# alexandre01/deepsvg

Hardware: AMD Instinct MI355X
Metric: SVG icons/sec (train step) hierarchical_ordered d=256 (higher is better)
Workload: dtype bf16; 1 GPU; hierarchical_ordered (Hierarchical, use_vae=False) G=8 S=30 d_model=256 ff=512 H=8 L=4x4; full train step = forward + SVGLoss + backward + grad-clip 1.0 + AdamW; dropout 0.1; global_batch=512, batch_per_gpu=512, parallelism=dp1, hip_graph=True, encoder_layout=packed (valid tokens only, exact)

## Files before the change

deepsvg_amd/csrc/gemm.hip:

```cpp
#include "mfma_frag.h"
#include "../../include/dsvg.h"
#include "gemm_common.h"
int dsvg_gemm_group_flush(hipStream_t st);
#include <map>
#include <mutex>
#include <vector>

template <typename T>
__global__ void gemm_naive_kernel(dsvg_gemm_desc p, int k_begin, int k_end, float* part, float* rs) {
    long long idx = (long long)blockIdx.x * blockDim.x + threadIdx.x;
    if (idx >= (long long)p.M * p.N) return;
    int m = (int)(idx / p.N), n = (int)(idx % p.N);
    const T* A = (const T*)p.A;
    const T* B = (const T*)p.B;
    DropCtx adc = drop_make(p.a_drop_p, p.seed, p.a_drop_site);
    float acc = 0.f, asum = 0.f;
    for (int k = k_begin; k < k_end; ++k) {
        float a, b;
        if (p.a_kc) {
            a = Elem<T>::ld(A + (size_t)m * p.lda + k);
            a *= drop_mult(adc, (uint64_t)m * p.a_drop_ld + k);
        } else {
            a = Elem<T>::ld(A + (size_t)k * p.lda + m);
            a *= drop_mult(adc, (uint64_t)k * p.a_drop_ld + m);
// ... 549 lines not shown
    if (int rc = dsvg_gemm_group_flush(st)) return rc;
    if (hipMemsetAsync(out, 0, (size_t)n * sizeof(float), st) != hipSuccess) { dsvg_set_error("defer_zero: hipMemsetAsync failed"); return -1; }
    return 0;
}

int dsvg_reduce_partials_mixed(const float* part, int64_t P, int64_t stride, int64_t n, int64_t n_bf16, float* out,
                               int32_t accumulate, hipStream_t st) {
    if (n <= 0) return 0;
    const bool vec = !(n & 3) && !(stride & 3) && !((uintptr_t)part & 15) && !((uintptr_t)out & 15) && !(n_bf16 & 3);
    {
        DeferTableOfQueues& t = defer_queues();
        std::lock_guard<std::mutex> lk(t.mu);
        auto it = t.by_stream.find(st);
        if (it != t.by_stream.end()) {
            DeferQueue& d = it->second;
            if (!d.q.empty() && defer_overlaps(d, out, n)) {
                int rc = defer_flush_locked(d, st);
                if (rc) return rc;
            }
            static const bool unaligned_ok = !(getenv("DSVG_DEFER_MORE") && atoi(getenv("DSVG_DEFER_MORE")) == 0);
            if (d.scope && (vec || (unaligned_ok && n_bf16 == 0)) && n < (1ll << 30) && P < (1ll << 30)) {
                d.q.push_back(DeferSeg{part, out, (long long)stride, (int)n, (int)n_bf16, (int)P, 0, accumulate, 0});
                return 0;
            }
        }
    }
    if (int rc = dsvg_gemm_group_flush(st)) return rc;
    if (n_bf16 > 0 && !vec) { dsvg_set_error("reduce_partials: bf16 partials need 16-byte aligned, 4-column-multiple data"); return -1; }
    const long long cols = vec ? n / 4 : n;
    const bool wide = cols >= 64 * 128 || P <= 16;
#define DSVG_RP(V, X, B) hipLaunchKernelGGL((reduce_partials_strided_kernel<V, X, B>), dim3(dsvg_cdiv(cols, X)), dim3(256), 0, \
                                            st, part, (long long)P, (long long)stride, (long long)n, out, accumulate,      \
                                            (long long)n_bf16)
    const bool narrow = !vec && n_bf16 == 0 && cols <= 4 && P > 64;
    if (n_bf16 > 0) { if (wide) DSVG_RP(4, 64, true); else DSVG_RP(4, 16, true); }
    else if (vec) { if (wide) DSVG_RP(4, 64, false); else DSVG_RP(4, 16, false); }
    else if (narrow) DSVG_RP(1, 4, false);
    else     { if (wide) DSVG_RP(1, 64, false); else DSVG_RP(1, 16, false); }
#undef DSVG_RP
    DSVG_LAUNCH_CHECK("reduce_partials");
    return 0;
}

constexpr int CS_ROWS_MIN = 16, CS_ROWS_MAX = 1024;
template <typename T>
__global__ __launch_bounds__(256) void colsum_kernel(const T* __restrict__ A, long long lda, long long M, int N,
                                                     float* __restrict__ part, float drop_p, uint32_t site,
                                                     const uint64_t* seed, int cpb, int vec_ok, int rows_per_block) {
    constexpr int VEC = 16 / (int)sizeof(T);
    __shared__ float red[256][VEC + 1];
    const DropCtx dc = drop_make(drop_p, seed, site);
    const int cl = threadIdx.x % cpb, rg = threadIdx.x / cpb, nrg = 256 / cpb;
    const int c0 = (blockIdx.y * cpb + cl) * VEC;
    const long long r0 = (long long)blockIdx.x * rows_per_block;
    const long long r1 = min(M, r0 + rows_per_block);
    float acc[VEC];
#pragma unroll
    for (int e = 0; e < VEC; ++e) acc[e] = 0.f;
    if (c0 < N) {
        if (vec_ok && c0 + VEC <= N) {
            for (long long r = r0 + rg; r < r1; r += nrg) {
                float v[VEC];
                if (VEC == 4) {
                    float t[4];
                    Elem<T>::ld4(A + r * lda + c0, t);
#pragma unroll
                    for (int e = 0; e < 4; ++e) v[e % VEC] = t[e];
                } else {
                    float t0[4], t1[4];
                    Elem<T>::ld4(A + r * lda + c0, t0);
                    Elem<T>::ld4(A + r * lda + c0 + 4, t1);
#pragma unroll
                    for (int e = 0; e < 4; ++e) { v[e] = t0[e]; v[(e + 4) % VEC] = t1[e]; }
                }
                if (VEC == 8 && dc.on && !(N & 7)) {
                    float m8[8];
                    drop_mult8(dc, (uint64_t)r * N + c0, m8);
#pragma unroll
                    for (int e = 0; e < VEC; ++e) acc[e] += v[e] * m8[e % 8];
                } else {
#pragma unroll
                    for (int e = 0; e < VEC; ++e) acc[e] += v[e] * drop_mult(dc, (uint64_t)r * N + c0 + e);
                }
            }
        } else {
            for (long long r = r0 + rg; r < r1; r += nrg)
#pragma unroll
                for (int e = 0; e < VEC; ++e)
                    if (c0 + e < N) acc[e] += Elem<T>::ld(A + r * lda + c0 + e) * drop_mult(dc, (uint64_t)r * N + c0 + e);
        }
    }
#pragma unroll
    for (int e = 0; e < VEC; ++e) red[threadIdx.x][e] = acc[e];
    __syncthreads();
    if (rg == 0 && c0 < N) {
#pragma unroll
        for (int e = 0; e < VEC; ++e) {
            if (c0 + e < N) {
                float s = 0.f;
                for (int g = 0; g < nrg; ++g) s += red[g * cpb + cl][e];
                part[(long long)blockIdx.x * N + c0 + e] = s;
            }
        }
    }
}

extern "C" int64_t dsvg_gemm_workspace_bytes(int32_t M, int32_t N, int32_t split_k) {
    if (split_k <= 1) return 0;
    return (int64_t)split_k * (int64_t)dsvg_splitk_slice(M, N, true) * (int64_t)sizeof(float);
}

extern "C" int dsvg_reduce_partials(const float* partial, int64_t P, int64_t n, float* out,
                                    int32_t accumulate, void* stream) {
    DSVG_CHECK_ARG(partial && out && P >= 0 && n >= 0, "reduce_partials: bad args");
    return dsvg_reduce_partials_strided(partial, P, n, n, out, accumulate, (hipStream_t)stream);
}

extern "C" int64_t dsvg_colsum_workspace_bytes(int64_t M, int32_t N) {
    return (int64_t)dsvg_cdiv(M, CS_ROWS_MIN) * N * (int64_t)sizeof(float);
}

extern "C" int dsvg_colsum(int32_t dtype, const void* A, int64_t lda, int64_t M, int32_t N, float* out,
                           int32_t accumulate, float drop_p, uint32_t drop_site, const uint64_t* seed,
                           float* workspace, int64_t workspace_bytes, void* stream) {
    DSVG_CHECK_ARG(A && out && M > 0 && N > 0, "colsum: bad args");
    DSVG_CHECK_ARG(workspace && workspace_bytes >= dsvg_colsum_workspace_bytes(M, N),
                   "colsum: workspace too small (%lld < %lld)", (long long)workspace_bytes,
                   (long long)dsvg_colsum_workspace_bytes(M, N));
    hipStream_t st = (hipStream_t)stream;
    DSVG_CHECK_ARG(dtype == DSVG_F32 || dtype == DSVG_BF16, "colsum: bad dtype %d", dtype);
    const int vec = dtype == DSVG_F32 ? 4 : 8;
    const int chunks = dsvg_cdiv(N, vec);
    int cpb = 8;
    while (cpb < 64 && cpb < chunks) cpb *= 2;
    const int vec_ok = !(lda % vec) && !((uintptr_t)A & 15);
    const int col_blocks = dsvg_cdiv(chunks, cpb);
    long long rpb = M / max(1, 1024 / col_blocks);
    rpb = rpb < CS_ROWS_MIN ? CS_ROWS_MIN : (rpb > CS_ROWS_MAX ? CS_ROWS_MAX : rpb);
    const int nb = dsvg_cdiv(M, rpb);
    dim3 grid(nb, col_blocks);
    if (dtype == DSVG_F32)
        hipLaunchKernelGGL(colsum_kernel<float>, grid, dim3(256), 0, st, (const float*)A, (long long)lda,
                           (long long)M, N, workspace, drop_p, drop_site, seed, cpb, vec_ok, (int)rpb);
    else
        hipLaunchKernelGGL(colsum_kernel<bf16_t>, grid, dim3(256), 0, st, (const bf16_t*)A, (long long)lda,
                           (long long)M, N, workspace, drop_p, drop_site, seed, cpb, vec_ok, (int)rpb);
    DSVG_LAUNCH_CHECK("colsum");
    return dsvg_reduce_partials(workspace, nb, N, out, accumulate, stream);
}

int dsvg_gemm_bf16_launch(const dsvg_gemm_desc& d, int k_chunk, int nsplit, float* part, float* rs_part,
                          hipStream_t st, int* part_is_bf16);

extern "C" int dsvg_gemm(const dsvg_gemm_desc* dp, void* stream) {
    DSVG_CHECK_ARG(dp, "gemm: null desc");
    dsvg_gemm_desc d = *dp;
    hipStream_t st = (hipStream_t)stream;
    DSVG_CHECK_ARG(d.dtype == DSVG_F32 || d.dtype == DSVG_BF16, "gemm: bad dtype %d", d.dtype);
    DSVG_CHECK_ARG(d.M > 0 && d.N > 0 && d.K > 0, "gemm: bad shape %d %d %d", d.M, d.N, d.K);
    DSVG_CHECK_ARG(d.A && d.B && d.C, "gemm: null operand");
    DSVG_CHECK_ARG((d.drop_p <= 0.f && d.a_drop_p <= 0.f) || d.seed, "gemm: dropout needs a seed pointer");
    if (d.dtype == DSVG_F32) d.c_f32 = 1;
    const int split = d.split_k > 1 ? d.split_k : 1;
    float* part = nullptr;
    int k_chunk = d.K;
    if (split > 1) {
        DSVG_CHECK_ARG(d.c_f32, "gemm: split_k needs fp32 output");
        DSVG_CHECK_ARG(!d.bias && !d.res && !d.gate && d.act == 0 && d.drop_p <= 0.f,
                       "gemm: split_k does not support an epilogue");
        DSVG_CHECK_ARG(d.workspace && d.workspace_bytes >= dsvg_gemm_workspace_bytes(d.M, d.N, split),
                       "gemm: split_k workspace too small");
        DSVG_CHECK_ARG(d.ldc == d.N, "gemm: split_k needs a dense C (ldc == N)");
        part = d.workspace;
        k_chunk = ((d.K + split - 1) / split + 63) / 64 * 64;
    }
    int nsplit = (d.K + k_chunk - 1) / k_chunk;
    if (split > 1 && (split % 8) == 0) nsplit = split;
    DSVG_CHECK_ARG(!d.rowsum || part, "gemm: rowsum needs split_k > 1");
    float* rs_part = d.rowsum ? part + (size_t)d.M * d.N : nullptr;
    const size_t slice = dsvg_splitk_slice(d.M, d.N, d.rowsum != nullptr);

    int part_bf16 = 0;
    bool use_naive = d.impl == 1;
    if (d.dtype == DSVG_F32) {
        if ((d.lda & 3) || (d.ldb & 3) || ((uintptr_t)d.A & 15) || ((uintptr_t)d.B & 15)) use_naive = true;
    } else {
        const int Kp = (d.K + 7) / 8 * 8;
        if ((d.lda & 7) || (d.ldb & 7) || ((uintptr_t)d.A & 15) || ((uintptr_t)d.B & 15)) use_naive = true;
        if ((d.a_kc && d.lda < Kp) || (d.b_kc && d.ldb < Kp)) use_naive = true;
        if (!d.a_kc && d.lda < ((d.M + 7) / 8) * 8) use_naive = true;
        if (!d.b_kc && d.ldb < ((d.N + 7) / 8) * 8) use_naive = true;
    }
    if (use_naive) {
        const long long total = (long long)d.M * d.N;
        for (int z = 0; z < nsplit; ++z) {
            const int kb = z * k_chunk, ke = min(d.K, kb + k_chunk);
            float* pz = part ? part + (size_t)z * slice : nullptr;
            float* rz = rs_part ? rs_part + (size_t)z * slice : nullptr;
            if (d.dtype == DSVG_F32)
                hipLaunchKernelGGL(gemm_naive_kernel<float>, dim3(dsvg_cdiv(total, 256)), dim3(256), 0, st, d, kb, ke, pz, rz);
            else
                hipLaunchKernelGGL(gemm_naive_kernel<bf16_t>, dim3(dsvg_cdiv(total, 256)), dim3(256), 0, st, d, kb, ke, pz, rz);
        }
        DSVG_LAUNCH_CHECK("gemm_naive");
    } else if (d.dtype == DSVG_F32) {
        const int tiles_m = dsvg_cdiv(d.M, BM), tiles_n = dsvg_cdiv(d.N, BN);
        const int nwg = tiles_m * tiles_n;
        dim3 grid(nwg, nsplit);
        if (nsplit > 1 && (nsplit % 8) == 0) grid = dim3(nwg * nsplit, 1);
#define DSVG_F32V(AK, BK)                                                                                              \
    do {                                                                                                               \
        if (rs_part) hipLaunchKernelGGL((gemm_f32_mfma_kernel<AK, BK, true>), grid, dim3(256), 0, st, d, tiles_n, nwg, \
                                        k_chunk, part, rs_part);                                                       \
        else hipLaunchKernelGGL((gemm_f32_mfma_kernel<AK, BK, false>), grid, dim3(256), 0, st, d, tiles_n, nwg,        \
                                k_chunk, part, rs_part);                                                               \
    } while (0)
        if (d.a_kc && d.b_kc) DSVG_F32V(true, true);
        else if (d.a_kc && !d.b_kc) DSVG_F32V(true, false);
        else if (!d.a_kc && d.b_kc) DSVG_F32V(false, true);
        else DSVG_F32V(false, false);
#undef DSVG_F32V
        DSVG_LAUNCH_CHECK("gemm_f32_mfma");
    } else {
        int rc = dsvg_gemm_bf16_launch(d, k_chunk, nsplit, part, rs_part, st, &part_bf16);
        if (rc) return rc;
    }
    if (part && part_bf16) {
        const int64_t mn = (int64_t)d.M * d.N;
        if (rs_part && d.rowsum == (float*)d.C + mn && !(d.M & 3))
            return dsvg_reduce_partials_mixed(part, nsplit, (int64_t)slice, mn + d.M, mn, (float*)d.C, d.accumulate, st);
        int rc = dsvg_reduce_partials_mixed(part, nsplit, (int64_t)slice, mn, mn, (float*)d.C, d.accumulate, st);
        if (rc) return rc;
        if (rs_part) return dsvg_reduce_partials_strided(rs_part, nsplit, (int64_t)slice, d.M, d.rowsum, d.accumulate, st);
        return 0;
    }
    if (part) {
        const int64_t mn = (int64_t)d.M * d.N;
        if (rs_part && d.rowsum == (float*)d.C + mn)
            return dsvg_reduce_partials_strided(part, nsplit, (int64_t)slice, mn + d.M, (float*)d.C, d.accumulate, st);
        int rc = dsvg_reduce_partials_strided(part, nsplit, (int64_t)slice, mn, (float*)d.C, d.accumulate, st);
        if (rc) return rc;
        if (rs_part) return dsvg_reduce_partials_strided(rs_part, nsplit, (int64_t)slice, d.M, d.rowsum, d.accumulate, st);
    }
    return 0;
}
```

deepsvg_amd/csrc/gemm_bf16.h:

```cpp
#pragma once
#include "dsvg_common.h"
#include "../../include/dsvg.h"

enum {
    EPI_GENERIC = 0,
    EPI_BIAS = 1,
    EPI_BIAS_RES_DROP = 2,
    EPI_BIAS_RELU_DROP = 3,
    EPI_GATE = 4,
    EPI_PARTIAL = 5,
};

bool dsvg_gemm_bf16_glds_try(const dsvg_gemm_desc& d, int epi, dim3 grid, int tiles_n, int nwg, int k_chunk,
                             float* part, float* rs_part, int mode, hipStream_t st, int* part_is_bf16);
int dsvg_gemm_group_flush(hipStream_t st);
```

deepsvg_amd/csrc/gemm_bf16_glds.hip:

```cpp
#include "gemm_bf16.h"
#include "mfma_frag.h"
#include <map>
#include <mutex>
#include <vector>

namespace {

constexpr int GBM = 128, GBN = 128, GBK = 64;
constexpr int IMG = 128 * 64;

__device__ __forceinline__ void dma_step8(const char* a0, const char* a1, const char* a2, const char* a3, const char* b0,
                                          const char* b1, const char* b2, const char* b3, uint32_t lds_a, uint32_t lds_b) {
    uint32_t keep;
    asm volatile(
        "s_mov_b32 %0, m0\n\t"
        "s_mov_b32 m0, %9\n\t"
        "s_nop 0\n\t"
        "global_load_lds_dwordx4 %1, off\n\t"
        "s_add_u32 m0, m0, 0x400\n\t"
        "s_nop 0\n\t"
        "global_load_lds_dwordx4 %2, off\n\t"
        "s_add_u32 m0, m0, 0x400\n\t"
        "s_nop 0\n\t"
        "global_load_lds_dwordx4 %3, off\n\t"
        "s_add_u32 m0, m0, 0x400\n\t"
        "s_nop 0\n\t"
        "global_load_lds_dwordx4 %4, off\n\t"
        "s_mov_b32 m0, %10\n\t"
        "s_nop 0\n\t"
        "global_load_lds_dwordx4 %5, off\n\t"
        "s_add_u32 m0, m0, 0x400\n\t"
        "s_nop 0\n\t"
        "global_load_lds_dwordx4 %6, off\n\t"
        "s_add_u32 m0, m0, 0x400\n\t"
        "s_nop 0\n\t"
        "global_load_lds_dwordx4 %7, off\n\t"
        "s_add_u32 m0, m0, 0x400\n\t"
        "s_nop 0\n\t"
        "global_load_lds_dwordx4 %8, off\n\t"
        "s_mov_b32 m0, %0"
        : "=&s"(keep)
        : "v"(a0), "v"(a1), "v"(a2), "v"(a3), "v"(b0), "v"(b1), "v"(b2), "v"(b3), "s"(lds_a), "s"(lds_b)
        : "memory", "scc");
}

template <bool AKC, bool BKC, int EPI, int NST>
__device__ __forceinline__ void glds_body(const dsvg_gemm_desc& p, int tiles_n, int nwg_mn, int k_chunk, float* part,
                                          float* rs_part, int mode, int part_bf16, int bid, int bid_y) {
    __shared__ __attribute__((aligned(1024))) bf16_t smem_static[NST <= 2 ? NST * 2 * IMG : 8];
    extern __shared__ __attribute__((aligned(1024))) bf16_t smem_dynamic[];
    bf16_t* const smem = NST <= 2 ? smem_static : smem_dynamic;

    const int xcd = bid % 8, local = bid / 8;
    int wgid, kz;
    if (mode == 1) {
        wgid = local % nwg_mn;
        kz = (local / nwg_mn) * 8 + xcd;
    } else {
        const int q8 = nwg_mn / 8, r8 = nwg_mn % 8;
        wgid = (xcd < r8 ? xcd * (q8 + 1) : r8 * (q8 + 1) + (xcd - r8) * q8) + local;
        kz = bid_y;
    }
    const int tile_m = wgid / tiles_n, tile_n = wgid % tiles_n;
    const int m0 = tile_m * GBM, n0 = tile_n * GBN;
    const int k_begin = kz * k_chunk;
    const int k_end = min(p.K, k_begin + k_chunk);

    const int tid = threadIdx.x;
    const int lane = tid & 63;
    const int wave = __builtin_amdgcn_readfirstlane(tid >> 6);
    const int wm = wave >> 1, wn = wave & 1;
    const int h = lane >> 5;

    uint32_t offa[4], offb[4];
#pragma unroll
    for (int i = 0; i < 4; ++i) {
        const int piece = wave * 4 + i;
        if (AKC) {
            const int r = piece * 8 + (lane >> 3);
            const int c = (lane & 7) ^ ((r >> 1) & 7);
            offa[i] = (uint32_t)(((size_t)min(m0 + r, p.M - 1) * p.lda + 8 * c) * 2);
        } else {
            const int kr = piece * 4 + (lane >> 4);
            const int c = (lane & 15) ^ ((lane >> 4) << 2);
            offa[i] = (uint32_t)(((size_t)kr * p.lda + min(m0 + 8 * c, ((p.M + 7) & ~7) - 8)) * 2);
        }
        if (BKC) {
            const int r = piece * 8 + (lane >> 3);
            const int c = (lane & 7) ^ ((r >> 1) & 7);
            offb[i] = (uint32_t)(((size_t)min(n0 + r, p.N - 1) * p.ldb + 8 * c) * 2);
        } else {
            const int kr = piece * 4 + (lane >> 4);
            const int c = (lane & 15) ^ ((lane >> 4) << 2);
            offb[i] = (uint32_t)(((size_t)kr * p.ldb + min(n0 + 8 * c, p.N - 8)) * 2);
        }
    }
    auto stage = [&](int k0, int buf) {
        const char* ab = (const char*)p.A + (AKC ? (size_t)k0 * 2 : (size_t)k0 * p.lda * 2);
        const char* bb = (const char*)p.B + (BKC ? (size_t)k0 * 2 : (size_t)k0 * p.ldb * 2);
        bf16_t* da = smem + buf * 2 * IMG + wave * 2048;
        bf16_t* db = da + IMG;
#pragma unroll
        for (int i = 0; i < 4; ++i) {
            __builtin_amdgcn_global_load_lds(DSVG_GLB_PTR(ab + offa[i]), DSVG_LDS_PTR(da + i * 512), 16, 0, 0);
            __builtin_amdgcn_global_load_lds(DSVG_GLB_PTR(bb + offb[i]), DSVG_LDS_PTR(db + i * 512), 16, 0, 0);
        }
    };

    uint32_t fk[4];
#pragma unroll
    for (int kk = 0; kk < 4; ++kk) fk[kk] = (uint32_t)(((lane & 31) * 64 + 8 * ((2 * kk + h) ^ ((lane >> 1) & 7))) * 2);
    const int g = lane >> 4, q = lane & 15;
    auto tr_off = [&](int w, int it) -> uint32_t {
        const int krow = 8 * (g >> 1) + (q >> 2);
        const int chunk = (8 * w + 4 * it + 2 * (g & 1) + ((q & 3) >> 1)) ^ (((q >> 2) & 3) << 2);
        return (uint32_t)((krow * 128 + 8 * chunk + 4 * (q & 1)) * 2);
    };
    const uint32_t ta0 = tr_off(wm, 0), ta1 = tr_off(wm, 1), tb0 = tr_off(wn, 0), tb1 = tr_off(wn, 1);

    auto frag_kc = [&](const char* img, int w, int it, int kk) -> bf16x8 {
        Frag8 f;
        f.u = *reinterpret_cast<const uint4*>(img + (w * 64 + it * 32) * 128 + fk[kk]);
        return f.v;
    };
    auto frag_tr = [&](const char* img, uint32_t off, int kk) -> bf16x8 {
        Frag8 f;
        f.h[0] = __builtin_amdgcn_ds_read_tr16_b64_v4i16((shortx4 __attribute__((address_space(3)))*)(img + off + kk * 4096));
        f.h[1] = __builtin_amdgcn_ds_read_tr16_b64_v4i16(
            (shortx4 __attribute__((address_space(3)))*)(img + off + kk * 4096 + 1024));
        return f.v;
    };

    if (EPI != EPI_PARTIAL && (part_bf16 & 16)) {
        const size_t span = (BKC ? (size_t)p.N * p.ldb : (size_t)p.K * p.ldb) * 2;
        const unsigned n_pc = (unsigned)((span + 4095) >> 12);
        const size_t off = (size_t)(((unsigned)bid >> 3) % n_pc) * 4096 + (size_t)wave * 1024 + (size_t)lane * 16;
        const char* src = (const char*)p.B + (off + 16 <= span ? off : span - 16);
        const uint32_t dst = __builtin_amdgcn_readfirstlane((uint32_t)(uintptr_t)DSVG_LDS_PTR(smem) + (uint32_t)wave * 4096u);
        uint32_t keep;
        asm volatile(
            "s_mov_b32 %0, m0\n\t"
            "s_mov_b32 m0, %2\n\t"
            "s_nop 0\n\t"
            "global_load_lds_dwordx4 %1, off\n\t"
            "s_mov_b32 m0, %0"
            : "=&s"(keep) : "v"(src), "s"(dst) : "memory");
    }

    floatx16 acc00, acc01, acc10, acc11;
#pragma unroll
    for (int r = 0; r < 16; ++r) { acc00[r] = 0.f; acc01[r] = 0.f; acc10[r] = 0.f; acc11[r] = 0.f; }
    const bool do_rs = (EPI == EPI_PARTIAL) && rs_part != nullptr && tile_n == 0;
    float rs0 = 0.f, rs1 = 0.f;
    auto rowsum8 = [](const bf16x8& f, float s) -> float {
        typedef __bf16 bf16x2 __attribute__((ext_vector_type(2)));
        Frag8 t;
        t.v = f;
        const uint32_t w[4] = {t.u.x, t.u.y, t.u.z, t.u.w};
        const bf16x2 one = __builtin_bit_cast(bf16x2, 0x3f803f80u);
#pragma unroll
        for (int e = 0; e < 4; ++e) s = __builtin_amdgcn_fdot2_f32_bf16(__builtin_bit_cast(bf16x2, w[e]), one, s, false);
        return s;
    };

    auto compute = [&](int buf) {
        const char* ia = (const char*)(smem + buf * 2 * IMG);
        const char* ib = ia + IMG * 2;
#pragma unroll
        for (int kk = 0; kk < GBK / 16; ++kk) {
            bf16x8 a0, a1, b0, b1;
            if (AKC) { a0 = frag_kc(ia, wm, 0, kk); a1 = frag_kc(ia, wm, 1, kk); }
            else     { a0 = frag_tr(ia, ta0, kk);   a1 = frag_tr(ia, ta1, kk); }
            if (BKC) { b0 = frag_kc(ib, wn, 0, kk); b1 = frag_kc(ib, wn, 1, kk); }
            else     { b0 = frag_tr(ib, tb0, kk);   b1 = frag_tr(ib, tb1, kk); }
            acc00 = __builtin_amdgcn_mfma_f32_32x32x16_bf16(b0, a0, acc00, 0, 0, 0);
            acc01 = __builtin_amdgcn_mfma_f32_32x32x16_bf16(b0, a1, acc01, 0, 0, 0);
            acc10 = __builtin_amdgcn_mfma_f32_32x32x16_bf16(b1, a0, acc10, 0, 0, 0);
            acc11 = __builtin_amdgcn_mfma_f32_32x32x16_bf16(b1, a1, acc11, 0, 0, 0);
            if (EPI == EPI_PARTIAL && do_rs && (kk >> 1) == wn) { rs0 = rowsum8(a0, rs0); rs1 = rowsum8(a1, rs1); }
        }
    };

    if (NST == 4) {
        const uint32_t lds0 = (uint32_t)(uintptr_t)DSVG_LDS_PTR(smem) + wave * 4096;
        auto issue = [&](int s) {
            const int k0 = k_begin + s * GBK;
            const char* ab = (const char*)p.A + (AKC ? (size_t)k0 * 2 : (size_t)k0 * p.lda * 2);
            const char* bb = (const char*)p.B + (BKC ? (size_t)k0 * 2 : (size_t)k0 * p.ldb * 2);
            const uint32_t la = __builtin_amdgcn_readfirstlane(lds0 + (uint32_t)(s & 3) * (2 * IMG * 2));
            dma_step8(ab + offa[0], ab + offa[1], ab + offa[2], ab + offa[3], bb + offb[0], bb + offb[1], bb + offb[2],
                      bb + offb[3], la, la + IMG * 2);
        };
        const int n_steps = (k_end - k_begin + GBK - 1) / GBK;
        for (int s = 0; s < 3 && s < n_steps; ++s) issue(s);
        for (int s = 0; s < n_steps; ++s) {
            const int ahead = min(n_steps - 1, s + 2) - s;
            if (ahead >= 2) asm volatile("s_waitcnt vmcnt(16)" ::: "memory");
            else if (ahead == 1) asm volatile("s_waitcnt vmcnt(8)" ::: "memory");
            else asm volatile("s_waitcnt vmcnt(0)" ::: "memory");
            __builtin_amdgcn_s_barrier();
            if (s + 3 < n_steps) issue(s + 3);
            compute(s & 3);
        }
    } else if (NST == 1) {
// ... 56 lines not shown
            if (wn == 0 && h == 0) {
                rs0 += rsx[wm * 64 + (lane & 31)];
                rs1 += rsx[wm * 64 + 32 + (lane & 31)];
                if (mrow < p.M) rs_part[(size_t)kz * slice + mrow] = rs0;
                if (mrow + 32 < p.M) rs_part[(size_t)kz * slice + mrow + 32] = rs1;
            }
        }
        return;
    }

    constexpr bool has_res = EPI == EPI_BIAS_RES_DROP;
    constexpr bool has_gate = EPI == EPI_GATE;
    constexpr bool relu = EPI == EPI_BIAS_RELU_DROP;
    constexpr bool may_drop = EPI == EPI_BIAS_RES_DROP || EPI == EPI_BIAS_RELU_DROP;
    const DropCtx dc = drop_make(may_drop ? p.drop_p : 0.f, p.seed, p.drop_site);
    const bool has_bias = !has_gate && p.bias != nullptr;
    const bool bias_al = (reinterpret_cast<uintptr_t>(p.bias) & 15) == 0;
    const bool n_aligned = !(p.N & 7);

    auto tile16 = [&](const floatx16& c, int jn, int im, uint4 (&pk)[2], int (&nvalid)[2]) {
        const int m = mrow + 32 * im;
        uint32_t x[4][4];
#pragma unroll
        for (int gq = 0; gq < 4; ++gq)
#pragma unroll
            for (int e = 0; e < 4; ++e) x[gq][e] = __float_as_uint(c[4 * gq + e]);
#pragma unroll
        for (int e = 0; e < 4; ++e) {
            auto s01 = __builtin_amdgcn_permlane32_swap(x[0][e], x[1][e], false, false);
            auto s23 = __builtin_amdgcn_permlane32_swap(x[2][e], x[3][e], false, false);
            x[0][e] = s01[0]; x[1][e] = s01[1]; x[2][e] = s23[0]; x[3][e] = s23[1];
        }
#pragma unroll
        for (int e = 0; e < 4; ++e) {
            auto s02 = __builtin_amdgcn_permlane32_swap(x[0][e], x[2][e], false, false);
            auto s13 = __builtin_amdgcn_permlane32_swap(x[1][e], x[3][e], false, false);
            x[0][e] = s02[0]; x[2][e] = s02[1]; x[1][e] = s13[0]; x[3][e] = s13[1];
        }
        const int n16 = ncol + 32 * jn + 16 * h;
#pragma unroll
        for (int cb = 0; cb < 2; ++cb) {
            float v[8];
#pragma unroll
            for (int e = 0; e < 4; ++e) { v[e] = __uint_as_float(x[2 * cb][e]); v[4 + e] = __uint_as_float(x[2 * cb + 1][e]); }
            const int nb = n16 + 8 * cb;
            const int nv = (m < p.M && nb < p.N) ? min(8, p.N - nb) : 0;
            nvalid[cb] = nv;
            if (nv == 0) { pk[cb] = make_uint4(0u, 0u, 0u, 0u); continue; }
            if (has_bias) {
                if (nv == 8 && bias_al) {
                    const float4 b0 = *reinterpret_cast<const float4*>(p.bias + nb);
                    const float4 b1 = *reinterpret_cast<const float4*>(p.bias + nb + 4);
                    v[0] += b0.x; v[1] += b0.y; v[2] += b0.z; v[3] += b0.w;
                    v[4] += b1.x; v[5] += b1.y; v[6] += b1.z; v[7] += b1.w;
                } else {
#pragma unroll
                    for (int e = 0; e < 8; ++e) v[e] += e < nv ? p.bias[nb + e] : 0.f;
                }
            }
            if (relu) {
#pragma unroll
                for (int e = 0; e < 8; ++e) v[e] = fmaxf(v[e], 0.f);
            }
            if (has_gate) {
                float gv[8];
                const bf16_t* gp = (const bf16_t*)p.gate + (size_t)m * p.ldgate + nb;
                if (nv == 8) unpack8(*reinterpret_cast<const uint4*>(gp), gv);
                else {
#pragma unroll
                    for (int e = 0; e < 8; ++e) gv[e] = e < nv ? bf2f(gp[e]) : 0.f;
                }
#pragma unroll
                for (int e = 0; e < 8; ++e) v[e] = gv[e] > 0.f ? v[e] * p.gate_scale : 0.f;
            }
            float rv[8];
            if (has_res) {
                const bf16_t* rp = (const bf16_t*)p.res + (size_t)m * p.ldres + nb;
                if (nv == 8) unpack8(*reinterpret_cast<const uint4*>(rp), rv);
                else {
#pragma unroll
                    for (int e = 0; e < 8; ++e) rv[e] = e < nv ? bf2f(rp[e]) : 0.f;
                }
                if (p.res_pre) {
#pragma unroll
                    for (int e = 0; e < 8; ++e) v[e] += rv[e];
                }
            }
            if (may_drop && dc.on) {
                float dm[8];
                if (n_aligned) {
                    drop_mult8(dc, (uint64_t)m * p.N + nb, dm);
                } else {
#pragma unroll
                    for (int e = 0; e < 8; ++e) dm[e] = drop_mult(dc, (uint64_t)m * p.N + nb + e);
                }
#pragma unroll
                for (int e = 0; e < 8; ++e) v[e] *= dm[e];
            }
            if (has_res && !p.res_pre) {
#pragma unroll
                for (int e = 0; e < 8; ++e) v[e] += rv[e];
            }
            pk[cb] = pack8(v);
        }
    };
    auto put8 = [&](bf16_t* cp, const uint4& v, int nv) {
        if (nv == 8) { *reinterpret_cast<uint4*>(cp) = v; return; }
        const uint32_t w[4] = {v.x, v.y, v.z, v.w};
#pragma unroll
        for (int e = 0; e < 8; ++e)
            if (e < nv) cp[e] = (bf16_t)((e & 1) ? (w[e >> 1] >> 16) : (w[e >> 1] & 0xffffu));
    };
    auto row_block = [&](const floatx16& c0, const floatx16& c1, int im) {
        uint4 pk0[2], pk1[2];
        int nv0[2], nv1[2];
        tile16(c0, 0, im, pk0, nv0);
        tile16(c1, 1, im, pk1, nv1);
        bf16_t* cp = (bf16_t*)p.C + (size_t)(mrow + 32 * im) * p.ldc + ncol + 16 * h;
        put8(cp, pk0[0], nv0[0]);
        put8(cp + 8, pk0[1], nv0[1]);
        put8(cp + 32, pk1[0], nv1[0]);
        put8(cp + 40, pk1[1], nv1[1]);
    };
    row_block(acc00, acc10, 0);
    row_block(acc01, acc11, 1);
}

template <bool AKC, bool BKC, int EPI, int NST, int OCC>
__global__ __launch_bounds__(256, NST == 1 ? OCC : 2) void gemm_bf16_glds_kernel(dsvg_gemm_desc p, int tiles_n, int nwg_mn,
                                                                              int k_chunk, float* part, float* rs_part,
                                                                              int mode, int part_bf16) {
    glds_body<AKC, BKC, EPI, NST>(p, tiles_n, nwg_mn, k_chunk, part, rs_part, mode, part_bf16, (int)blockIdx.x, (int)blockIdx.y);
}

constexpr int GROUP_MAX = 16;
struct WgItem {
    const void* A; const void* B; float* part; float* rs_part;
    int M, N, K, tiles_n, nwg_mn, k_chunk, mode, part_bf16, first_block, grid_x;
    long long lda, ldb;
};
struct WgTable { WgItem it[GROUP_MAX]; int n; };
static_assert(sizeof(WgTable) <= 3600, "the problem table must fit the kernel-argument segment");

__global__ __launch_bounds__(256, 2) void gemm_bf16_wgrad_group_kernel(const WgTable t) {
    int g = 0;
    while (g + 1 < t.n && (int)blockIdx.x >= t.it[g + 1].first_block) ++g;
    const WgItem& w = t.it[g];
    dsvg_gemm_desc p;
    p.A = w.A; p.B = w.B; p.M = w.M; p.N = w.N; p.K = w.K; p.lda = w.lda; p.ldb = w.ldb;
    const int local = (int)blockIdx.x - w.first_block;
    glds_body<false, false, EPI_PARTIAL, 4>(p, w.tiles_n, w.nwg_mn, w.k_chunk, w.part, w.rs_part, w.mode, w.part_bf16,
                                            local % w.grid_x, local / w.grid_x);
}

struct GroupQueue {
    int scope = 0;
    std::vector<WgItem> q;
};
struct GroupQueues {
    std::mutex mu;
    std::map<hipStream_t, GroupQueue> by_stream;
};
GroupQueues& group_queues() { static GroupQueues g; return g; }

int group_launch_locked(GroupQueue& gq, hipStream_t st) {
    size_t at = 0;
    while (at < gq.q.size()) {
        WgTable t;
        int blocks = 0, k = 0;
        for (; k < GROUP_MAX && at < gq.q.size(); ++k, ++at) {
            t.it[k] = gq.q[at];
            t.it[k].first_block = blocks;
            blocks += gq.q[at].first_block;
        }
        t.n = k;
        const size_t lds = (size_t)4 * 2 * IMG * sizeof(bf16_t);
        static bool once = false;
        if (!once) {
            (void)hipFuncSetAttribute((const void*)gemm_bf16_wgrad_group_kernel, hipFuncAttributeMaxDynamicSharedMemorySize,
                                      (int)lds);
            once = true;
        }
        hipLaunchKernelGGL(gemm_bf16_wgrad_group_kernel, dim3(blocks), dim3(256), lds, st, t);
    }
    gq.q.clear();
    return 0;
}

template <bool AKC, bool BKC, int EPI>
void launch(const dsvg_gemm_desc& d, dim3 grid, int tiles_n, int nwg, int k_chunk, float* part, float* rs_part, int mode,
            int nst, hipStream_t st, int pbf = 0) {
    static const int occ = getenv("DSVG_GEMM_OCC") ? atoi(getenv("DSVG_GEMM_OCC")) : 4;
    static const int w_warm = getenv("DSVG_GEMM_WARM") ? atoi(getenv("DSVG_GEMM_WARM")) : 0;
    if (EPI != EPI_PARTIAL && w_warm) pbf |= 16;
    if (nst == 4) {
        const size_t lds = (size_t)4 * 2 * IMG * sizeof(bf16_t);
        static bool once = false;
        if (!once) {
            (void)hipFuncSetAttribute((const void*)gemm_bf16_glds_kernel<AKC, BKC, EPI, 4, 4>,
                                      hipFuncAttributeMaxDynamicSharedMemorySize, (int)lds);
            once = true;
        }
        hipLaunchKernelGGL((gemm_bf16_glds_kernel<AKC, BKC, EPI, 4, 4>), grid, dim3(256), lds, st, d, tiles_n, nwg, k_chunk,
                           part, rs_part, mode, pbf);
    } else if (nst == 2)
        hipLaunchKernelGGL((gemm_bf16_glds_kernel<AKC, BKC, EPI, 2, 4>), grid, dim3(256), 0, st, d, tiles_n, nwg, k_chunk,
                           part, rs_part, mode, pbf);
    else if (occ == 5)
        hipLaunchKernelGGL((gemm_bf16_glds_kernel<AKC, BKC, EPI, 1, 5>), grid, dim3(256), 0, st, d, tiles_n, nwg, k_chunk,
                           part, rs_part, mode, pbf);
    else
        hipLaunchKernelGGL((gemm_bf16_glds_kernel<AKC, BKC, EPI, 1, 4>), grid, dim3(256), 0, st, d, tiles_n, nwg, k_chunk,
                           part, rs_part, mode, pbf);
}

}

bool dsvg_gemm_bf16_glds_try(const dsvg_gemm_desc& d, int epi, dim3 grid, int tiles_n, int nwg, int k_chunk, float* part,
                             float* rs_part, int mode, hipStream_t st, int* part_is_bf16) {
    static const bool pbf_on = !(getenv("DSVG_SPLITK_BF16") && atoi(getenv("DSVG_SPLITK_BF16")) == 0);
    static const bool disabled = getenv("DSVG_GEMM_NOGLDS") != nullptr;
    static const int nst_env = getenv("DSVG_GEMM_STAGES") ? atoi(getenv("DSVG_GEMM_STAGES")) : 1;
    if (disabled || d.impl == 2 || mode == 2 || d.a_drop_p > 0.f) return false;
    static const int deep_wgs = getenv("DSVG_GEMM_DEEP_WGS") ? atoi(getenv("DSVG_GEMM_DEEP_WGS")) : 256;
    const long long n_wgs = (long long)grid.x * grid.y * grid.z;
    const int nst = d.impl == 6 ? 4 : (d.impl == 3 ? 2 : (d.impl == 4 ? 1 : (n_wgs <= deep_wgs ? 4 : nst_env)));
    if ((d.K % GBK) || (part && (k_chunk % GBK))) return false;
    if ((d.lda & 7) || (d.ldb & 7) || ((uintptr_t)d.A & 15) || ((uintptr_t)d.B & 15)) return false;
    if (!d.a_kc && d.M < 8) return false;
    if (!d.b_kc && ((d.N & 7) || d.N < 8)) return false;
    if (d.M < 1 || d.N < 1) return false;
    const size_t span_a = d.a_kc ? (size_t)d.M * d.lda : (size_t)GBK * d.lda + d.M;
    const size_t span_b = d.b_kc ? (size_t)d.N * d.ldb : (size_t)GBK * d.ldb + d.N;
    if (span_a * 2 >= (1ull << 32) || span_b * 2 >= (1ull << 32)) return false;
    if (part) {
        if (((uintptr_t)part & 15) || (d.N & 3)) return false;
        if (!d.a_kc && !d.b_kc) {
            const int pbf = (pbf_on && part_is_bf16 && !(d.N & 7)) ? 1 : 0;
            if (nst == 4 && grid.z == 1) {
                GroupQueues& G = group_queues();
                std::lock_guard<std::mutex> lk(G.mu);
                auto it = G.by_stream.find(st);
                if (it != G.by_stream.end() && it->second.scope) {
                    WgItem w;
                    w.A = d.A; w.B = d.B; w.part = part; w.rs_part = rs_part;
                    w.M = d.M; w.N = d.N; w.K = d.K; w.tiles_n = tiles_n; w.nwg_mn = nwg; w.k_chunk = k_chunk; w.mode = mode;
                    w.part_bf16 = pbf; w.first_block = (int)(grid.x * grid.y); w.grid_x = (int)grid.x;
                    w.lda = d.lda; w.ldb = d.ldb;
                    it->second.q.push_back(w);
                    if (part_is_bf16) *part_is_bf16 = pbf;
                    return true;
                }
            }
            launch<false, false, EPI_PARTIAL>(d, grid, tiles_n, nwg, k_chunk, part, rs_part, mode, nst, st, pbf);
            if (part_is_bf16) *part_is_bf16 = pbf;
            return true;
        }
        return false;
    }
    if (d.bias && ((uintptr_t)d.bias & 3)) return false;
    if (d.a_kc && d.b_kc) {
        if (epi == EPI_BIAS) launch<true, true, EPI_BIAS>(d, grid, tiles_n, nwg, k_chunk, part, rs_part, mode, nst, st);
        else if (epi == EPI_BIAS_RES_DROP) launch<true, true, EPI_BIAS_RES_DROP>(d, grid, tiles_n, nwg, k_chunk, part, rs_part, mode, nst, st);
        else if (epi == EPI_BIAS_RELU_DROP) launch<true, true, EPI_BIAS_RELU_DROP>(d, grid, tiles_n, nwg, k_chunk, part, rs_part, mode, nst, st);
        else return false;
        return true;
    }
    if (d.a_kc && !d.b_kc) {
        if (epi == EPI_BIAS) launch<true, false, EPI_BIAS>(d, grid, tiles_n, nwg, k_chunk, part, rs_part, mode, nst, st);
        else if (epi == EPI_GATE) launch<true, false, EPI_GATE>(d, grid, tiles_n, nwg, k_chunk, part, rs_part, mode, nst, st);
        else return false;
        return true;
    }
    return false;
}

int dsvg_gemm_group_flush(hipStream_t st) {
    GroupQueues& G = group_queues();
    std::lock_guard<std::mutex> lk(G.mu);
    auto it = G.by_stream.find(st);
    if (it == G.by_stream.end() || it->second.q.empty()) return 0;
    const int rc = group_launch_locked(it->second, st);
    hipError_t e = hipGetLastError();
    if (e != hipSuccess) { dsvg_set_error("gemm group: launch failed: %s", hipGetErrorString(e)); return -2; }
    return rc;
}

extern "C" int dsvg_gemm_group_scope(int32_t on, void* stream) {
    hipStream_t st = (hipStream_t)stream;
    {
        GroupQueues& G = group_queues();
        std::lock_guard<std::mutex> lk(G.mu);
        if (on) { G.by_stream[st].scope = 1; return 0; }
        auto it = G.by_stream.find(st);
        if (it == G.by_stream.end()) return 0;
        it->second.scope = 0;
    }
    const int rc = dsvg_gemm_group_flush(st);
    {
        GroupQueues& G = group_queues();
        std::lock_guard<std::mutex> lk(G.mu);
        auto it = G.by_stream.find(st);
        if (it != G.by_stream.end() && it->second.q.empty() && !it->second.scope) G.by_stream.erase(it);
    }
    return rc;
}
```

deepsvg_amd/csrc/layernorm.hip:

```cpp
#include "dsvg_common.h"
#include "../../include/dsvg.h"

constexpr int LN_MAXV_MAX = 4;
constexpr int LN_MAX_BLOCKS = 1024;

template <typename T, int LN_MAXV>
__global__ __launch_bounds__(256) void ln_fwd_kernel(const T* __restrict__ x, const float* __restrict__ gamma,
                                                     const float* __restrict__ beta, T* __restrict__ y,
                                                     float* __restrict__ mean, float* __restrict__ rstd,
                                                     long long rows, int d, float eps) {
    const int lane = threadIdx.x & 63;
    const int wave = threadIdx.x >> 6;
    const int nv = d / 256 + ((d % 256) ? 1 : 0);
    float4 g4[LN_MAXV], b4[LN_MAXV];
#pragma unroll
    for (int i = 0; i < LN_MAXV; ++i) {
        const int c = min(i * 256 + lane * 4, d - 4);
        g4[i] = *reinterpret_cast<const float4*>(gamma + c);
        b4[i] = *reinterpret_cast<const float4*>(beta + c);
    }
    for (long long row = (long long)blockIdx.x * 4 + wave; row < rows; row += (long long)gridDim.x * 4) {
        const T* xr = x + row * d;
        float v[LN_MAXV][4];
        float s = 0.f;
#pragma unroll
        for (int i = 0; i < LN_MAXV; ++i) {
            const int c = i * 256 + lane * 4;
            if (i < nv && c < d) {
                Elem<T>::ld4(xr + c, v[i]);
                s += v[i][0] + v[i][1] + v[i][2] + v[i][3];
            } else {
                v[i][0] = v[i][1] = v[i][2] = v[i][3] = 0.f;
            }
        }
        const float mu = wave_sum(s) / (float)d;
        float s2 = 0.f;
#pragma unroll
        for (int i = 0; i < LN_MAXV; ++i) {
            const int c = i * 256 + lane * 4;
            if (i < nv && c < d) {
#pragma unroll
                for (int e = 0; e < 4; ++e) { const float t = v[i][e] - mu; s2 += t * t; }
            }
        }
        const float var = wave_sum(s2) / (float)d;
        const float rs = rsqrtf(var + eps);
        if (lane == 0) { mean[row] = mu; rstd[row] = rs; }
        T* yr = y + row * d;
#pragma unroll
        for (int i = 0; i < LN_MAXV; ++i) {
            const int c = i * 256 + lane * 4;
            if (i < nv && c < d) {
                const float4 g = g4[i];
                const float4 b = b4[i];
                float o[4];
                o[0] = (v[i][0] - mu) * rs * g.x + b.x;
                o[1] = (v[i][1] - mu) * rs * g.y + b.y;
                o[2] = (v[i][2] - mu) * rs * g.z + b.z;
                o[3] = (v[i][3] - mu) * rs * g.w + b.w;
                Elem<T>::st4(yr + c, o);
            }
        }
    }
}

template <typename T, int LN_MAXV>
__global__ __launch_bounds__(256) void ln_bwd_kernel(const T* dy, const T* __restrict__ x,
                                                     const float* __restrict__ mean, const float* __restrict__ rstd,
                                                     const float* __restrict__ gamma, const T* res,
                                                     T* dx, float* __restrict__ part,
                                                     long long rows, int d, T* dxm, float drop_p,
                                                     const uint64_t* __restrict__ seed, uint32_t site) {
    const DropCtx dmc = drop_make(dxm ? drop_p : 0.f, seed, site);
    extern __shared__ float red_raw[];
    const int nvec = d / 4 + 1;
    auto red = [&](int w, int k, int vec, int e) -> float& { return red_raw[((w * 2 + k) * nvec + vec) * 4 + e]; };
    const int lane = threadIdx.x & 63;
    const int wave = threadIdx.x >> 6;
    const int nv = d / 256 + ((d % 256) ? 1 : 0);
    float ag[LN_MAXV][4], ab[LN_MAXV][4];
#pragma unroll
    for (int i = 0; i < LN_MAXV; ++i)
#pragma unroll
        for (int e = 0; e < 4; ++e) { ag[i][e] = 0.f; ab[i][e] = 0.f; }

    float4 g4[LN_MAXV];
#pragma unroll
    for (int i = 0; i < LN_MAXV; ++i) g4[i] = *reinterpret_cast<const float4*>(gamma + min(i * 256 + lane * 4, d - 4));
    for (long long row = (long long)blockIdx.x * 4 + wave; row < rows; row += (long long)gridDim.x * 4) {
        const float mu = mean[row], rs = rstd[row];
        float xh[LN_MAXV][4], gd[LN_MAXV][4], rv[LN_MAXV][4];
        float c1 = 0.f, c2 = 0.f;
#pragma unroll
        for (int i = 0; i < LN_MAXV; ++i) {
            const int c = i * 256 + lane * 4;
            if (i < nv && c < d) {
                float xv[4], dv[4];
                Elem<T>::ld4(x + row * d + c, xv);
                Elem<T>::ld4(dy + row * d + c, dv);
                if (res) Elem<T>::ld4(res + row * d + c, rv[i]);
                const float4 g = g4[i];
                const float gg[4] = {g.x, g.y, g.z, g.w};
#pragma unroll
                for (int e = 0; e < 4; ++e) {
                    xh[i][e] = (xv[e] - mu) * rs;
                    gd[i][e] = gg[e] * dv[e];
                    c1 += gd[i][e];
                    c2 += gd[i][e] * xh[i][e];
                    ag[i][e] += dv[e] * xh[i][e];
                    ab[i][e] += dv[e];
                }
            } else {
#pragma unroll
                for (int e = 0; e < 4; ++e) { xh[i][e] = 0.f; gd[i][e] = 0.f; }
            }
        }
        c1 = wave_sum(c1) / (float)d;
        c2 = wave_sum(c2) / (float)d;
#pragma unroll
        for (int i = 0; i < LN_MAXV; ++i) {
            const int c = i * 256 + lane * 4;
            if (i < nv && c < d) {
                float o[4];
#pragma unroll
                for (int e = 0; e < 4; ++e) o[e] = rs * (gd[i][e] - c1 - xh[i][e] * c2);
                if (res) {
#pragma unroll
                    for (int e = 0; e < 4; ++e) o[e] += rv[i][e];
                }
                Elem<T>::st4(dx + row * d + c, o);
                if (dxm) {
                    const uint64_t id4 = (uint64_t)row * (uint64_t)d + (uint64_t)c;
                    float mm[4] = {1.f, 1.f, 1.f, 1.f};
                    if (dmc.on) {
                        const uint32_t hg = drop_group(dmc, id4 >> 3);
                        const uint32_t wb = ((uint32_t)id4 & 4u) ? 2u : 0u;
                        const uint32_t w0 = drop_word(hg, wb), w1 = drop_word(hg, wb + 1u);
                        mm[0] = (w0 & 0xffffu) < dmc.thresh ? 0.f : dmc.scale;
                        mm[1] = (w0 >> 16) < dmc.thresh ? 0.f : dmc.scale;
                        mm[2] = (w1 & 0xffffu) < dmc.thresh ? 0.f : dmc.scale;
                        mm[3] = (w1 >> 16) < dmc.thresh ? 0.f : dmc.scale;
                    }
                    float om[4];
#pragma unroll
                    for (int e = 0; e < 4; ++e) {
                        T t;
                        Elem<T>::st(&t, o[e]);
                        om[e] = Elem<T>::ld(&t) * mm[e];
                    }
                    Elem<T>::st4(dxm + row * d + c, om);
                }
            }
        }
    }
#pragma unroll
    for (int i = 0; i < LN_MAXV; ++i) {
        if (i < nv) {
#pragma unroll
            for (int e = 0; e < 4; ++e) {
                if (i * 256 + lane * 4 < d) {
                    red(wave, 0, i * 64 + lane, e) = ag[i][e];
                    red(wave, 1, i * 64 + lane, e) = ab[i][e];
                }
            }
        }
    }
    __syncthreads();
    float* pg = part + (size_t)blockIdx.x * 2 * d;
    for (int c = threadIdx.x; c < d; c += 256) {
        const int vec = c >> 2, e = c & 3;
        float sg = 0.f, sb = 0.f;
#pragma unroll
        for (int w = 0; w < 4; ++w) { sg += red(w, 0, vec, e); sb += red(w, 1, vec, e); }
        pg[c] = sg;
        pg[d + c] = sb;
    }
}

static int ln_grid(long long rows) {
    static const int cap = getenv("DSVG_LN_BLOCKS") ? atoi(getenv("DSVG_LN_BLOCKS")) : LN_MAX_BLOCKS;
    long long nb = (rows + 3) / 4;
    return (int)(nb < cap ? nb : cap);
}
static int ln_grid_fwd(long long rows) {
    long long nb = (rows + 3) / 4;
    return (int)(nb < 65536 ? nb : 65536);
}

extern "C" int dsvg_layernorm_fwd(int32_t dtype, const void* x, const float* gamma, const float* beta, void* y,
                                  float* mean, float* rstd, int64_t rows, int32_t d, float eps, void* stream) {
    DSVG_CHECK_ARG(x && gamma && beta && y && mean && rstd, "layernorm_fwd: null pointer");
    DSVG_CHECK_ARG(rows > 0 && d > 0 && (d % 4) == 0 && d <= 1024, "layernorm_fwd: bad shape rows=%lld d=%d",
                   (long long)rows, d);
    hipStream_t st = (hipStream_t)stream;
#define DSVG_LNF(TT, NV) hipLaunchKernelGGL((ln_fwd_kernel<TT, NV>), dim3(ln_grid_fwd(rows)), dim3(256), 0, st, \
                                            (const TT*)x, gamma, beta, (TT*)y, mean, rstd, (long long)rows, d, eps)
    if (dtype == DSVG_F32) { if (d <= 256) DSVG_LNF(float, 1); else if (d <= 512) DSVG_LNF(float, 2); else DSVG_LNF(float, 4); }
    else if (dtype == DSVG_BF16) { if (d <= 256) DSVG_LNF(bf16_t, 1); else if (d <= 512) DSVG_LNF(bf16_t, 2); else DSVG_LNF(bf16_t, 4); }
    else { dsvg_set_error("layernorm_fwd: bad dtype %d", dtype); return -1; }
#undef DSVG_LNF
    DSVG_LAUNCH_CHECK("layernorm_fwd");
    return 0;
}

extern "C" int64_t dsvg_layernorm_bwd_workspace_bytes(int64_t rows, int32_t d) {
    return (int64_t)ln_grid(rows) * 2 * d * (int64_t)sizeof(float);
}

static int ln_bwd_launch(int32_t dtype, const void* dy, const void* x, const float* mean, const float* rstd,
                         const float* gamma, const void* res, void* dx, float* dgamma, float* dbeta,
                         int32_t accumulate, int64_t rows, int32_t d, float* workspace,
                         int64_t workspace_bytes, void* dx_masked, float drop_p, uint32_t drop_site, const void* seed,
                         void* stream);

extern "C" int dsvg_layernorm_bwd(int32_t dtype, const void* dy, const void* x, const float* mean, const float* rstd,
                                  const float* gamma, const void* res, void* dx, float* dgamma, float* dbeta,
                                  int32_t accumulate, int64_t rows, int32_t d, float* workspace,
                                  int64_t workspace_bytes, void* stream) {
    return ln_bwd_launch(dtype, dy, x, mean, rstd, gamma, res, dx, dgamma, dbeta, accumulate, rows, d, workspace,
                         workspace_bytes, nullptr, 0.f, 0u, nullptr, stream);
}

extern "C" int dsvg_layernorm_bwd_masked(int32_t dtype, const void* dy, const void* x, const float* mean, const float* rstd,
                                         const float* gamma, const void* res, void* dx, float* dgamma, float* dbeta,
                                         int32_t accumulate, int64_t rows, int32_t d, float* workspace,
                                         int64_t workspace_bytes, void* dx_masked, float drop_p, uint32_t drop_site,
                                         const void* seed, void* stream) {
    DSVG_CHECK_ARG(dx_masked && dx_masked != dx, "layernorm_bwd_masked: needs a second output buffer");
    DSVG_CHECK_ARG(!(drop_p > 0.f) || seed, "layernorm_bwd_masked: dropout needs a seed");
    return ln_bwd_launch(dtype, dy, x, mean, rstd, gamma, res, dx, dgamma, dbeta, accumulate, rows, d, workspace,
                         workspace_bytes, dx_masked, drop_p, drop_site, seed, stream);
}

static int ln_bwd_launch(int32_t dtype, const void* dy, const void* x, const float* mean, const float* rstd,
                         const float* gamma, const void* res, void* dx, float* dgamma, float* dbeta,
                         int32_t accumulate, int64_t rows, int32_t d, float* workspace,
                         int64_t workspace_bytes, void* dx_masked, float drop_p, uint32_t drop_site, const void* seed,
                         void* stream) {
    DSVG_CHECK_ARG(dy && x && mean && rstd && gamma && dx && dgamma && dbeta, "layernorm_bwd: null pointer");
    DSVG_CHECK_ARG(rows > 0 && d > 0 && (d % 4) == 0 && d <= 1024, "layernorm_bwd: bad shape");
    DSVG_CHECK_ARG(workspace && workspace_bytes >= dsvg_layernorm_bwd_workspace_bytes(rows, d),
                   "layernorm_bwd: workspace too small");
    hipStream_t st = (hipStream_t)stream;
    const int nb = ln_grid(rows);
    const size_t lds = (size_t)4 * 2 * (d / 4 + 1) * 4 * sizeof(float);
#define DSVG_LNB(TT, NV) hipLaunchKernelGGL((ln_bwd_kernel<TT, NV>), dim3(nb), dim3(256), lds, st, (const TT*)dy, \
                                            (const TT*)x, mean, rstd, gamma, (const TT*)res, (TT*)dx, workspace,  \
                                            (long long)rows, d, (TT*)dx_masked, drop_p, (const uint64_t*)seed, drop_site)
    if (dtype == DSVG_F32) { if (d <= 256) DSVG_LNB(float, 1); else if (d <= 512) DSVG_LNB(float, 2); else DSVG_LNB(float, 4); }
    else if (dtype == DSVG_BF16) { if (d <= 256) DSVG_LNB(bf16_t, 1); else if (d <= 512) DSVG_LNB(bf16_t, 2); else DSVG_LNB(bf16_t, 4); }
    else { dsvg_set_error("layernorm_bwd: bad dtype %d", dtype); return -1; }
#undef DSVG_LNB
    DSVG_LAUNCH_CHECK("layernorm_bwd");
    if (dbeta == dgamma + d)
        return dsvg_reduce_partials_strided(workspace, nb, 2 * (int64_t)d, 2 * (int64_t)d, dgamma, accumulate, st);
    int rc = 0;
    rc = dsvg_reduce_partials_strided(workspace, nb, 2 * (int64_t)d, d, dgamma, accumulate, st);
    if (rc) return rc;
    rc = dsvg_reduce_partials_strided(workspace + d, nb, 2 * (int64_t)d, d, dbeta, accumulate, st);
    return rc;
}
```

deepsvg_amd/functional.py:

```python
import math
import contextlib
import functools
import os

import torch

from . import ops

FFN_MIN_ROWS = int(os.environ.get("DSVG_FFN_MIN_ROWS", "16384"))
ATTN_MIN_ROWS = int(os.environ.get("DSVG_ATTN_MIN_ROWS", "16384"))
FFN_GATE_DW2 = os.environ.get("DSVG_FFN_GATE_DW2", "1") != "0"

LN_BWD_MASKED = os.environ.get("DSVG_LN_BWD_MASKED", "1") != "0"
DEFER_MORE = os.environ.get("DSVG_DEFER_MORE", "1") != "0"
HEAD_KPAD = os.environ.get("DSVG_HEAD_KPAD", "1") != "0"
GS_STACK = os.environ.get("DSVG_GS_STACK", "1") != "0"
_ATTN_VALU = os.environ.get("DSVG_ATTN_VALU") is not None
_ATTN_MFMA_MIN_S = int(os.environ.get("DSVG_ATTN_MFMA_MIN_S", "2"))
GS_REMAINDER = int(os.environ.get("DSVG_GS_REMAINDER", "512"))
SEQ_ROUND = 2048
HEAD_FUSED = os.environ.get("DSVG_HEAD_FUSED", "0") != "0"

_NULL_CTX = contextlib.nullcontext()

class Runtime:

    def __init__(self, dtype=torch.float32, seed=None, store=None, training=False, defer=False):
        self.dtype = dtype
        self.defer = bool(defer)
        self.seed = seed
        self.store = store
        self.training = training
        self.masked = {}
        self.last_layer_gs = False
        self.stack_group = None
        self.path_stage = False
        self.cond_grad = {}

    def cond_grad_block(self, z, rows):
        if z is None or z.dim() != 2 or z.stride(1) != 1 or z.dtype != torch.bfloat16:
            return None
        w, ld = z.shape[1], z.stride(0)
        if ld <= w or ld % w or w % 8 or w > 512:
            return None
        i = (z.storage_offset() % ld) // w
        if (z.storage_offset() % ld) % w:
            return None
        base = z.data_ptr() - i * w * z.element_size()
        key = (base, rows, ld)
        buf = self.cond_grad.get(key)
        if buf is None:
            if len(self.cond_grad) > 8:
                self.cond_grad.clear()
            buf = self.cond_grad[key] = torch.empty((rows, ld), dtype=z.dtype, device=z.device)
        return buf[:, i * w:(i + 1) * w]

    def deferring(self):
        return ops.DEFER if self.defer else _NULL_CTX

    def stack_group_begin(self):
        if self.stack_group is None:
            ops.GROUP.__enter__()
            self.stack_group = []
        return self.stack_group

    def stack_group_end(self):
        if self.stack_group is not None:
            ops.GROUP.__exit__(None, None, None)
            self.stack_group = None

    def deferring_tables(self):
        return ops.DEFER if self.defer and DEFER_MORE else _NULL_CTX

    def grouping(self):
        return ops.GROUP

    def p(self, rate):
        return float(rate) if (self.training and rate > 0.0) else 0.0

    def w(self, param):
        if self.dtype == torch.float32:
            return param.detach()
        if self.store is not None:
            v = self.store.lp(param)
            if v is not None:
                return v
        return param.detach().to(self.dtype)

    def grad_out(self, param):
        if self.store is not None:
            v = self.store.grad_view(param)
            if v is not None:
                return v
        return torch.empty(param.shape, dtype=torch.float32, device=param.device)


def _wgrad_tag():
    return ops.tag_default("wgrad") if ops.PROFILE_ON else _NULL_CTX


def _wgrad(rt, param, dy, x, *, a_drop_p=0.0, a_drop_site=0):
    out = rt.grad_out(param)
    n_out, k_in = param.shape
    T = dy.shape[0]
    with rt.deferring(), _wgrad_tag():
        ops.gemm(dy, x, a_kc=False, b_kc=False, out=out.view(n_out, k_in), a_drop_p=a_drop_p, a_drop_site=a_drop_site,
                 seed=rt.seed, split_k=ops.split_k_for(n_out, k_in, T))
    return out


def _wbgrad(rt, weight, bias, dy, x, blocks=None, *, out=None, split=None, defer=True):
    if split is None:
        split = ops.split_k_for(*weight.shape, dy.shape[0], target_blocks=blocks)
    dw, db = out if out is not None else (rt.grad_out(weight), rt.grad_out(bias))
    with (rt.deferring() if defer else _NULL_CTX), _wgrad_tag():
        if split > 1:
            ops.gemm(dy, x, a_kc=False, b_kc=False, out=dw, split_k=split, rowsum=db)
        else:
            ops.gemm(dy, x, a_kc=False, b_kc=False, out=dw)
            ops.colsum(dy, out=db)
    return dw, db


def _group_blocks(w):
    return 8 * -(-w.shape[0] // 128) * -(-w.shape[1] // 128)


def _bgrad(rt, param, dy, *, drop_p=0.0, drop_site=0):
    out = rt.grad_out(param)
    with rt.deferring():
        ops.colsum(dy, out=out, drop_p=drop_p, drop_site=drop_site, seed=rt.seed)
    return out


def _hand_masked(rt, dx, dxm, p, site):
    if len(rt.masked) > 8:
        rt.masked.clear()
    rt.masked[dx.data_ptr()] = (dxm, p, site, dx._version)


def _take_masked(rt, dx, p, site, rows=None):
    hit = rt.masked.pop(dx.data_ptr(), None)
    if hit is None:
        return None
    dxm, hp, hsite, ver = hit
    n = dx.shape[0] if rows is None else rows
    if (hp != p or hsite != site or dxm.dtype != dx.dtype or dxm.shape[0] < n or dxm.shape[1:] != dx.shape[1:]
            or dx._version != ver):
        return None
    return dxm[:n]


def _aligned2d(t, mult):
    if t.dim() == 2 and t.stride(1) == 1 and t.stride(0) % mult == 0 and t.data_ptr() % 16 == 0:
        return t
    rows, cols = t.shape
    ld = (cols + mult - 1) // mult * mult
    buf = torch.zeros((rows, ld), dtype=t.dtype, device=t.device)
    buf[:, :cols].copy_(t)
    return buf[:, :cols]


class LinearFn(torch.autograd.Function):

    @staticmethod
    def forward(ctx, rt, x, weight, bias, act, res, drop_rate, site, out_dtype):
        p = rt.p(drop_rate)
        dt = out_dtype or x.dtype
        n_out = weight.shape[0]
        mult = 4 if dt == torch.float32 else 8
        out = None
        if n_out % mult:
            ld = (n_out + mult - 1) // mult * mult
            out = torch.empty((x.shape[0], ld), dtype=dt, device=x.device)[:, :n_out]
        y = ops.gemm(x, rt.w(weight), bias=bias.detach() if bias is not None else None, act=act,
                     res=res, drop_p=p, drop_site=site, seed=rt.seed, out_dtype=out_dtype, out=out)
        ctx.rt, ctx.act, ctx.p, ctx.site = rt, act, p, site
        ctx.has_res = res is not None
        ctx.save_for_backward(x, weight, bias, y if act == ops.RELU else None)
        return y

    @staticmethod
    def backward(ctx, dy):
        rt = ctx.rt
        x, weight, bias, y = ctx.saved_tensors
        mult = 4 if rt.dtype == torch.float32 else 8
        dy = _aligned2d(dy.to(rt.dtype) if dy.dtype != rt.dtype else dy, mult)
        dres = dy if ctx.has_res else None
        if ctx.act == ops.RELU:
            assert not ctx.has_res, "relu with a fused residual cannot be differentiated from the saved output"
            scale = ops.keep_scale(ctx.p)
            dy_eff, a_drop_p_eff, a_site = ops.gate_mul(dy.contiguous(), y, scale), 0.0, 0
        else:
            dy_eff, a_drop_p_eff, a_site = dy, ctx.p, ctx.site
        dx = None
        if ctx.needs_input_grad[1]:
            dx = ops.gemm(dy_eff, rt.w(weight), b_kc=False, a_drop_p=a_drop_p_eff, a_drop_site=a_site, seed=rt.seed)
        if a_drop_p_eff == 0.0 and bias is not None:
            dw, db = _wbgrad(rt, weight, bias, dy_eff, x)
        else:
            dw = _wgrad(rt, weight, dy_eff, x, a_drop_p=a_drop_p_eff, a_drop_site=a_site)
            db = _bgrad(rt, bias, dy_eff, drop_p=a_drop_p_eff, drop_site=a_site) if bias is not None else None
        return None, dx, dw, db, None, dres, None, None, None


class ResBlockFn(torch.autograd.Function):

    @staticmethod
    def forward(ctx, rt, z, weight, bias):
        r = ops.gemm(z, rt.w(weight), bias=bias.detach(), act=ops.RELU)
        ctx.rt = rt
        ctx.save_for_backward(z, r, weight, bias)
        return ops.add(z, r)

    @staticmethod
    def backward(ctx, dout):
        rt = ctx.rt
        z, r, weight, bias = ctx.saved_tensors
        dout = dout.contiguous()
        dpre = ops.gate_mul(dout, r, 1.0)
        dw, db = _wbgrad(rt, weight, bias, dpre, z)
        dz = ops.gemm(dpre, rt.w(weight), b_kc=False, res=dout)
        return None, dz, dw, db


LATENT_FUSED = os.environ.get("DSVG_LATENT_FUSED", "1") != "0"


class LatentChainFn(torch.autograd.Function):

    @staticmethod
    def forward(ctx, rt, z, *wb):
        ws = [rt.w(w) for w in wb[0::2]]
        bs = [b.detach() for b in wb[1::2]]
        ctx.rt, ctx.n = rt, len(ws) - 1
        z = z.contiguous()
        if any(ctx.needs_input_grad):
            out, zs, rs = ops.latent_chain_fwd(z, ws, bs, train=True)
            ctx.save_for_backward(z, *zs, *rs, *wb)
        else:
            out = ops.latent_chain_fwd(z, ws, bs)
        return out

    @staticmethod
    def backward(ctx, dout):
        rt, n = ctx.rt, ctx.n
        saved = ctx.saved_tensors
        zin = [saved[0]] + list(saved[1:1 + n])
        rs = list(saved[1 + n:1 + 2 * n])
        wb = saved[1 + 2 * n:]
        dout = dout.contiguous()
        dz0, dpre = ops.latent_chain_bwd(dout, [rt.w(w) for w in wb[0::2]], rs)
        grads = []
        with rt.grouping():
            for i in range(n + 1):
                w, b = wb[2 * i], wb[2 * i + 1]
                grads += list(_wbgrad(rt, w, b, dpre[i] if i < n else dout, zin[i], _group_blocks(w)))
        return (None, dz0, *grads)


class LivePrefix(tuple):
    armed = False


def _live_rows(live, full_rows):
    if live is None or live[1] >= full_rows:
        return None
    return live


def _armed(live):
    if live is None or not getattr(live, "armed", True):
        return None
    return live
# ... 415 lines not shown
            xn1, mean1, rstd1 = ops.layernorm_fwd(x, n1w.detach(), n1b.detach())
            qkv = ops.gemm(xn1, rt.w(win), bias=bin_.detach())
            if causal:
                ao = ops.attention_fwd(qkv, key_mask, n_seq, S, n_heads, scale, p, site0, rt.seed, causal=True)
            else:
                ao = ops.attention_fwd(qkv, key_mask, n_seq, S, n_heads, scale, p, site0, rt.seed, seq_off=seq_off,
                                       tiles=tiles, **_path_kw(rt, S))
            x1 = ops.gemm(ao, rt.w(wo), bias=bo.detach(), res=x, drop_p=p, drop_site=site0 + 1, seed=rt.seed)
        ctx.tiles, ctx.causal = tiles, causal
        if z is not None and not z_fused:
            g = z.contiguous() if wg is None else ops.gemm(z, rt.w(wg), bias=bg.detach())
            ops.bcast_add_fwd_(x1, g, n_seq, S, p, site0 + 2, rt.seed)
        if l is not None:
            g2 = ops.gemm(l, rt.w(wg2), bias=bg2.detach())
            ops.bcast_add_fwd_(x1, g2, n_seq, S, p, site0 + 5, rt.seed)
        ffn = rt.store.ffn(w1) if (rt.store is not None and x.dtype == torch.bfloat16 and x.shape[0] >= FFN_MIN_ROWS) else None
        ctx.ffn_fused = ffn is not None
        if split:
            pass
        elif ffn is not None:
            mean2 = rstd2 = None
            with ops.tag("ffn"):
                if want_bwd:
                    x2, h, xn2, _rstd = ops.ffn_fwd(x1, ffn[0], ffn[2], b2.detach(), 1e-5, p, site0 + 3, site0 + 4, rt.seed,
                                                    train=True)
                else:
                    xn2 = h = None
                    x2 = ops.ffn_fwd(x1, ffn[0], ffn[2], b2.detach(), 1e-5, p, site0 + 3, site0 + 4, rt.seed)
        else:
            with ops.tag("ffn"):
                xn2, mean2, rstd2 = ops.layernorm_fwd(x1, n2w.detach(), n2b.detach())
                h = ops.gemm(xn2, rt.w(w1), bias=b1.detach(), act=ops.RELU, drop_p=p, drop_site=site0 + 3, seed=rt.seed)
                x2 = ops.gemm(h, rt.w(w2), bias=b2.detach(), res=x1, drop_p=p, drop_site=site0 + 4, seed=rt.seed)
        ctx.rt, ctx.n_seq, ctx.S, ctx.n_heads, ctx.p, ctx.site0, ctx.scale = rt, n_seq, S, n_heads, p, site0, scale
        assert seq_off is None or (z is None and l is None), "packed layout: no per-sequence conditioning adds"
        ctx.live = _live_rows(live, x.shape[0])
        assert ctx.live is None or (seq_off is None and key_mask is None and l is None)
        ctx.save_for_backward(x, key_mask, z, l, mean1, rstd1, xn1, qkv, ao, x1, mean2, rstd2, xn2, h,
                              n1w, n1b, win, bin_, wo, bo, n2w, n2b, w1, b1, w2, b2, wg, bg, wg2, bg2, seq_off)
        return x2

    @staticmethod
    def backward(ctx, dx2):
        rt, n_seq, S, H, p, s0 = ctx.rt, ctx.n_seq, ctx.S, ctx.n_heads, ctx.p, ctx.site0
        (x, key_mask, z, l, mean1, rstd1, xn1, qkv, ao, x1, mean2, rstd2, xn2, h,
         n1w, n1b, win, bin_, wo, bo, n2w, n2b, w1, b1, w2, b2, wg, bg, wg2, bg2, seq_off) = ctx.saved_tensors
        dx2 = dx2.contiguous()
        full_rows, n_seq_full = x.shape[0], n_seq
        live = _armed(ctx.live)
        dx2_masked = _take_masked(rt, dx2, p, s0 + 4, rows=(live[1] if live is not None else None)) if p > 0 else None
        if live is not None:
            n_seq, R = live
            (dx2, x, mean1, rstd1, xn1, qkv, ao, x1, mean2, rstd2, xn2, h) = (
                (t[:R] if t is not None else None) for t in (dx2, x, mean1, rstd1, xn1, qkv, ao, x1, mean2, rstd2, xn2, h))
        inv_keep = ops.keep_scale(p)
        dx1m = None
        if ctx.gs:
            gs = rt.store.gs(win)
            with rt.deferring(), ops.tag("gs"):
                (dx, dx1, dym, dpre, dx1m, dqkv, dn2w, dn2b, dn1w, dn1b, *dg_) = ops.gs_layer_bwd(
                    dx2, gs[1], x, mean1, rstd1, qkv, x1, mean2, rstd2, h, n1w.detach(), n2w.detach(), key_mask, n_seq, S,
                    ctx.scale, p, s0, rt.seed, want_dx1=False, dgamma2=rt.grad_out(n2w),
                    dbeta2=rt.grad_out(n2b), dgamma1=rt.grad_out(n1w), dbeta1=rt.grad_out(n1b), want_dg=z is not None)
            dz = dg = None
            if z is not None:
                dg = dg_[0]
                if wg is None:
                    dz = dg
                elif ctx.needs_input_grad[3]:
                    dz = ops.gemm(dg, rt.w(wg), b_kc=False)
            (dw2, db2), (dw1, db1), (dwo, dbo), (dwin, dbin), (dwg, dbg) = _gs_queue_wgrads(
                rt, ctx.first_in_stack, (w2, b2, dym, h), (w1, b1, dpre, xn2), (wo, bo, dx1m, ao), (win, bin_, dqkv, xn1),
                cond=(wg if z is not None else None, bg, dg, z))
            return (None, dx, None, dz, None, None, None, None, None, None,
                    dn1w, dn1b, dwin, dbin, dwo, dbo, dn2w, dn2b, dw1, db1, dw2, db2, dwg, dbg, None, None, None, None, None,
                    None, None, None)
        if ctx.ffn_fused:
            pb, _b1f, w2p = rt.store.ffn(w1)[1:]
            T = x1.shape[0]
            with ops.tag("ffn"):
                g2p = torch.empty((256, 512), dtype=torch.float32, device=x1.device)
                g1p = torch.empty((512, 256), dtype=torch.float32, device=x1.device)
                db1p = torch.empty(512, dtype=torch.float32, device=x1.device)
                db2 = rt.grad_out(b2)
                s2, s1 = ops.split_k_for(256, 512, T), ops.split_k_for(512, 256, T)
                hp, xh = h, xn2
                dym = dx2_masked if dx2_masked is not None else ops.drop_apply(dx2, p, s0 + 4, rt.seed)
                if (FFN_GATE_DW2 and s2 > 1 and dym.is_cuda and dym.dtype == torch.bfloat16
                        and dym.is_contiguous() and hp.is_contiguous() and w2p.is_contiguous()):
                    with rt.deferring():
                        dpre = ops.ffn_gate_dw2(dym, hp, w2p, inv_keep, g2p, db2, s2)
                else:
                    _wbgrad(rt, None, None, dym, hp, out=(g2p, db2), split=s2)
                    dpre = ops.gemm(dym, w2p, b_kc=False, gate=hp, gate_scale=inv_keep)
                _wbgrad(rt, None, None, dpre, xh, out=(g1p, db1p), split=s1)
                dx1 = ops.ffn_bwd_dx(dpre, x1, dx2, pb)
                dw1, db1, dw2 = rt.grad_out(w1), rt.grad_out(b1), rt.grad_out(w2)
                dn2w, dn2b = rt.grad_out(n2w), rt.grad_out(n2b)
                fin = (g1p, db1p, g2p, w1.detach(), n2w.detach(), n2b.detach(), dw1.detach(), db1.detach(), dw2.detach(),
                       dn2w.detach(), dn2b.detach())
                if rt.defer:
                    ops.ffn_wgrad_finish_deferred(*fin)
                else:
                    ops.ffn_wgrad_finish(*fin)
            del hp, dpre, xh, dym
        else:
            with ops.tag("ffn"):
                dx2m = dx2_masked if dx2_masked is not None else ops.drop_apply(dx2, p, s0 + 4, rt.seed)
                dw2, db2 = _wbgrad(rt, w2, b2, dx2m, h)
                dh = ops.gemm(dx2m, rt.w(w2), b_kc=False, gate=h, gate_scale=inv_keep)
                dw1, db1 = _wbgrad(rt, w1, b1, dh, xn2)
                dxn2 = ops.gemm(dh, rt.w(w1), b_kc=False)
                with rt.deferring():
                    dx1, dn2w, dn2b = ops.layernorm_bwd(dxn2, x1, mean2, rstd2, n2w.detach(), res=dx2,
                                                        dgamma=rt.grad_out(n2w), dbeta=rt.grad_out(n2b))
            del dx2m
        dz = dl = dwg = dbg = dwg2 = dbg2 = None
        if l is not None:
            dg2 = ops.bcast_add_bwd(dx1, n_seq, S, p, s0 + 5, rt.seed)
            dwg2, dbg2 = _wbgrad(rt, wg2, bg2, dg2, l)
            if ctx.needs_input_grad[4]:
                dl = ops.gemm(dg2, rt.w(wg2), b_kc=False)
        if z is not None:
            vec = dx1.dtype == torch.bfloat16 and dx1.is_contiguous() and dx1.shape[1] % 8 == 0 and dx1.shape[1] <= 512
            dg_out = rt.cond_grad_block(z, n_seq_full) if (wg is None and vec and dx1.data_ptr() % 16 == 0) else None
            if p > 0 and vec and n_seq * S <= dx1.shape[0] <= n_seq_full * S:
                dg, dx1m = ops.bcast_add_bwd(dx1, n_seq, S, p, s0 + 2, rt.seed, n_seq_out=n_seq_full, mask_site=s0 + 1, out=dg_out)
            else:
                dg = ops.bcast_add_bwd(dx1, n_seq, S, p, s0 + 2, rt.seed, n_seq_out=n_seq_full, out=dg_out)
            if wg is None:
                dz = dg
            else:
                dwg, dbg = _wbgrad(rt, wg, bg, dg, z)
                if ctx.needs_input_grad[3]:
                    dz = ops.gemm(dg, rt.w(wg), b_kc=False)
        if dx1m is None:
            dx1m = ops.drop_apply(dx1, p, s0 + 1, rt.seed)
        dwo, dbo = _wbgrad(rt, wo, bo, dx1m, ao)
        wob = None
        if (not _ATTN_VALU and S >= _ATTN_MFMA_MIN_S and _attn_fused_eligible(rt, x, x.shape[0], key_mask, H, ctx.causal)
                and ((seq_off is None and 16 < S <= 32 and x.shape[0] >= n_seq * S) or (seq_off is not None and ctx.tiles is not None))):
            wob = rt.store.attn_bwd(win)
        if wob is not None:
            dqkv = ops.attention_bwd_outproj(qkv, key_mask, dx1m, wob, n_seq, S, ctx.scale, p, s0, rt.seed, seq_off=seq_off,
                                             tiles=ctx.tiles)
        else:
            dao = ops.gemm(dx1m, rt.w(wo), b_kc=False)
            if ctx.causal:
                dqkv = ops.attention_bwd(qkv, key_mask, dao, n_seq, S, H, ctx.scale, p, s0, rt.seed, causal=True)
            else:
                dqkv = ops.attention_bwd(qkv, key_mask, dao, n_seq, S, H, ctx.scale, p, s0, rt.seed, seq_off=seq_off,
                                         tiles=ctx.tiles, **_path_kw(rt, S))
        del dx1m
        dwin, dbin = _wbgrad(rt, win, bin_, dqkv, xn1)
        dx_out = None
        if live is not None:
            dx_full = torch.empty((full_rows, x.shape[1]), dtype=x.dtype, device=x.device)
            dx_out = dx_full[:x.shape[0]]
        mk = (p, ctx.mask_below, rt.seed) if (ctx.mask_below is not None and p > 0) else None
        with rt.deferring():
            dxn1 = ops.gemm(dqkv, rt.w(win), b_kc=False)
            out = ops.layernorm_bwd(dxn1, x, mean1, rstd1, n1w.detach(), res=dx1, dx=dx_out,
                                    dgamma=rt.grad_out(n1w), dbeta=rt.grad_out(n1b), masked=mk)
            dx, dn1w, dn1b = out[:3]
        if live is not None:
            dx = dx_full
        if mk is not None:
            _hand_masked(rt, dx, out[3], p, ctx.mask_below)
        return (None, dx, None, dz, dl, None, None, None, None, None,
                dn1w, dn1b, dwin, dbin, dwo, dbo, dn2w, dn2b, dw1, db1, dw2, db2, dwg, dbg, dwg2, dbg2, None, None, None,
                None, None, None)


def gs_stack_eligible(rt, x, key_mask, n_seq, S, n_heads, n_layers, wins):
    return (GS_STACK and x.dim() == 2 and _gs_eligible(rt, x, key_mask, n_seq, S, n_heads)
            and 1 <= n_layers <= ops.GS_STACK_MAX and all(rt.store.gs(w) is not None for w in wins))


class GsStackFn(torch.autograd.Function):

    @staticmethod
    def forward(ctx, rt, x, key_mask, n_seq, S, n_heads, drop_rate, site0, n_layers, has_g, *tensors):
        p = rt.p(drop_rate)
        per = 13 if has_g else 12
        assert len(tensors) == per * n_layers
        scale = float(x.shape[1] // n_heads) ** -0.5
        want_bwd = any(ctx.needs_input_grad)
        layers = []
        for i in range(n_layers):
            n1w, n1b, win, bin_, wo, bo, n2w, n2b, w1, b1, w2, b2 = tensors[per * i:per * i + 12]
            layers.append(dict(img=rt.store.gs(win)[0], in_bias=bin_.detach(), out_bias=bo.detach(), b1=b1.detach(), b2=b2.detach(),
                               gamma1=n1w.detach(), beta1=n1b.detach(), gamma2=n2w.detach(), beta2=n2b.detach(),
                               site0=site0 + 8 * i, seq_add=tensors[per * i + 12] if has_g else None))
        with ops.tag("gs"):
            res = ops.gs_stack_fwd(x, layers, key_mask, n_seq, S, scale, 1e-5, p, rt.seed, train=want_bwd)
        rt.last_layer_gs = True
        ctx.rt, ctx.n_seq, ctx.S, ctx.p, ctx.site0, ctx.scale, ctx.n, ctx.has_g = rt, n_seq, S, p, site0, scale, n_layers, has_g
        if not want_bwd:
            return res[-1]
        saved = [x, key_mask]
        for r in res:
            saved += list(r)
        ctx.save_for_backward(*saved, *tensors)
        return res[-1][0]

    @staticmethod
    def backward(ctx, dx2):
        rt, n_seq, S, p, n, has_g = ctx.rt, ctx.n_seq, ctx.S, ctx.p, ctx.n, ctx.has_g
        sv = ctx.saved_tensors
        x, key_mask = sv[0], sv[1]
        acts = [sv[2 + 11 * i:2 + 11 * (i + 1)] for i in range(n)]
        tensors = sv[2 + 11 * n:]
        per = 13 if has_g else 12
        prm = [tensors[per * i:per * i + 12] for i in range(n)]
        layers = []
        for i in range(n):
            x2, mean1, rstd1, xn1, qkv, ao, x1, mean2, rstd2, xn2, h = acts[i]
            n1w, n1b, win, bin_, wo, bo, n2w, n2b, w1, b1, w2, b2 = prm[i]
            layers.append(dict(img=rt.store.gs(win)[1], x=x if i == 0 else acts[i - 1][0], mean1=mean1, rstd1=rstd1, qkv=qkv, x1=x1,
                               mean2=mean2, rstd2=rstd2, h=h, gamma1=n1w.detach(), gamma2=n2w.detach(), site0=ctx.site0 + 8 * i,
                               dgamma2=rt.grad_out(n2w), dbeta2=rt.grad_out(n2b), dgamma1=rt.grad_out(n1w),
                               dbeta1=rt.grad_out(n1b)))
        with rt.deferring(), ops.tag("gs"):
            dx, ops_, dgcat = ops.gs_stack_bwd(dx2.contiguous(), layers, key_mask, n_seq, S, ctx.scale, p, rt.seed, want_dg=has_g)
        grads = [None] * (per * n)
        for i in range(n - 1, -1, -1):
            x2, mean1, rstd1, xn1, qkv, ao, x1, mean2, rstd2, xn2, h = acts[i]
            n1w, n1b, win, bin_, wo, bo, n2w, n2b, w1, b1, w2, b2 = prm[i]
            dym, dpre, dx1m, dqkv = ops_[i]
            (dw2, db2), (dw1, db1), (dwo, dbo), (dwin, dbin), _ = _gs_queue_wgrads(
                rt, i == 0, (w2, b2, dym, h), (w1, b1, dpre, xn2), (wo, bo, dx1m, ao), (win, bin_, dqkv, xn1))
            L = layers[i]
            grads[per * i:per * i + 12] = [L["dgamma1"], L["dbeta1"], dwin, dbin, dwo, dbo, L["dgamma2"], L["dbeta2"], dw1, db1, dw2, db2]
            if has_g:
                grads[per * i + 12] = dgcat[:, 256 * i:256 * (i + 1)]
        return (None, dx, None, None, None, None, None, None, None, None, *grads)


class MaskedCEFn(torch.autograd.Function):

    @staticmethod
    def forward(ctx, logits2d, target, w, C_, group, count_fn):
        lse, sc = ops.masked_ce_fwd(logits2d, target, w, C_, group)
        if count_fn is not None:
            sc = torch.stack([sc[0], count_fn(sc[1].clone()).to(sc.dtype).reshape(())])
        ctx.C_, ctx.group = C_, group
        ctx.save_for_backward(logits2d, target, w, lse, sc)
        return sc

    @staticmethod
    def backward(ctx, dsc):
        logits2d, target, w, lse, sc = ctx.saved_tensors
        g = dsc[0:1].to(torch.float32).contiguous()
        mult = 4 if logits2d.dtype == torch.float32 else 8
        dlogits = ops.masked_ce_bwd(logits2d, target, w, lse, sc, g, 1.0, ctx.C_, ctx.group, pad_to=mult)
        return dlogits, None, None, None, None, None


class LossCombineFn(torch.autograd.Function):

    @staticmethod
    def forward(ctx, weights, *scs):
        out = ops.loss_combine_fwd([sc.contiguous() for sc in scs], weights)
        ctx.weights, ctx.device = tuple(float(w) for w in weights), out.device
        ctx.set_materialize_grads(False)
        return tuple(out.unbind(0))

    @staticmethod
    def backward(ctx, dtotal, *dterms):
        f32 = lambda t: None if t is None else t.reshape(1).to(torch.float32).contiguous()
        dsc = ops.loss_combine_bwd(f32(dtotal), [f32(t) for t in dterms], ctx.weights, ctx.device)
        return (None,) + tuple(dsc.unbind(0))


def _tail_is_own_bias_or_slack(st, weight, bias, n_read):
    ent, entb = st.index.get(id(weight)), st.index.get(id(bias))
    if ent is None:
        return False
    end_read = ent[0] + n_read
    for p in st.params:
        o, n, _shape = st.index[id(p)]
        if o >= ent[0] + ent[1] and o < end_read and p is not bias:
            return False
    return entb is None or entb[0] >= ent[0] + ent[1]


class ArgsHeadLossFn(torch.autograd.Function):

    @staticmethod
    def forward(ctx, rt, x, weight, bias, target, w, C_, group, count_fn, live, slot_lo=0, cmd_logits=None,
                cmd_weight=None, cmd_bias=None, cmd_target=None, cmd_w=None, cmd_count_fn=None):
        R = min(int(live[1]), x.shape[0])
        idx = live[0][:R]
        xc = ops.gather_groups(x, idx, R, 1)
        r0, r1 = slot_lo * C_, (slot_lo + group) * C_
        n_out = r1 - r0
        w_used = rt.w(weight)[r0:r1]
        b_used = bias.detach()[r0:r1]
        if HEAD_FUSED and b_used.data_ptr() % 16:
            b_used = b_used.clone()
        ctx.head_img = None
        if HEAD_FUSED and xc.dtype == torch.bfloat16 and xc.shape[1] == 256 and C_ >= 64 and n_out <= 3008:
            ctx.head_img = ops.head_pack(w_used if w_used.is_contiguous() else w_used.contiguous())
            logits_c = None
            lse, sc = ops.head_lse(xc, ctx.head_img, b_used, n_out, C_, target, w, tok_idx=idx)
        else:
            mult = 4 if xc.dtype == torch.float32 else (64 if HEAD_KPAD else 8)
            ld = (n_out + mult - 1) // mult * mult
            buf = torch.empty((R, ld), dtype=xc.dtype, device=xc.device)
            logits_c = buf[:, :n_out]
            ops.gemm(xc, w_used, bias=b_used, out=logits_c)
            lse, sc = ops.masked_ce_fwd(logits_c, target, w, C_, group, tok_idx=idx)
        ctx.b_used = b_used
        if count_fn is not None:
            sc = torch.stack([sc[0], count_fn(sc[1].clone()).to(sc.dtype).reshape(())])
        ctx.rt, ctx.C_, ctx.group, ctx.rows_full, ctx.rows_used = rt, C_, group, x.shape[0], (r0, r1)
# ... 75 lines not shown
```

deepsvg_amd/lib.py:

```python
import ctypes as C
import os

_HERE = os.path.dirname(os.path.abspath(__file__))
LIB_PATH = os.path.join(_HERE, "_lib", "libdsvg_hip.so")

DSVG_F32 = 0
DSVG_BF16 = 1
DSVG_I64 = 2
DSVG_RASTER_FILL, DSVG_RASTER_CULL = 1, 2
DSVG_RASTER_WIDE = 4
ABI_VERSION = 18

c_i32, c_i64, c_u32, c_f32 = C.c_int32, C.c_int64, C.c_uint32, C.c_float
vp = C.c_void_p


class GemmDesc(C.Structure):
    _fields_ = [
        ("dtype", c_i32), ("M", c_i32), ("N", c_i32), ("K", c_i32),
        ("A", vp), ("lda", c_i64), ("a_kc", c_i32),
        ("B", vp), ("ldb", c_i64), ("b_kc", c_i32),
        ("C", vp), ("ldc", c_i64), ("c_f32", c_i32),
        ("bias", vp),
        ("res", vp), ("ldres", c_i64), ("res_pre", c_i32),
        ("act", c_i32),
        ("gate", vp), ("ldgate", c_i64), ("gate_scale", c_f32),
        ("drop_p", c_f32), ("drop_site", c_u32),
        ("a_drop_p", c_f32), ("a_drop_site", c_u32), ("a_drop_ld", c_i64),
        ("seed", vp),
        ("accumulate", c_i32),
        ("split_k", c_i32), ("workspace", vp), ("workspace_bytes", c_i64),
        ("rowsum", vp),
        ("impl", c_i32),
    ]


class GsFwdLayer(C.Structure):
    _fields_ = [(n, vp) for n in ("packed_fwd_layer", "in_bias", "out_bias", "b1", "b2", "gamma1", "beta1", "gamma2", "beta2",
                                  "seq_add", "x2", "mean1", "rstd1", "xn1", "qkv", "ao", "x1", "mean2", "rstd2", "xn2", "h")] + [
        ("site0", c_u32), ("reserved_", c_u32)]


class GsBwdLayer(C.Structure):
    _fields_ = [(n, vp) for n in ("packed_bwd_layer", "x", "mean1", "rstd1", "qkv", "x1", "mean2", "rstd2", "h", "gamma1", "gamma2",
                                  "dx", "dx1", "dym", "dpre", "dx1m", "dqkv", "dg", "dgamma2", "dbeta2", "dgamma1", "dbeta1",
                                  "workspace")] + [("site0", c_u32), ("reserved_", c_u32)]


SIGNATURES = {
    "dsvg_last_error": (C.c_char_p, []),
    "dsvg_version": (c_i32, []),
    "dsvg_gemm": (c_i32, [C.POINTER(GemmDesc), vp]),
    "dsvg_gemm_workspace_bytes": (c_i64, [c_i32, c_i32, c_i32]),
    "dsvg_reduce_partials": (c_i32, [vp, c_i64, c_i64, vp, c_i32, vp]),
    "dsvg_defer_scope": (c_i32, [c_i32, vp]),
    "dsvg_flush_deferred": (c_i32, [vp]),
    "dsvg_defer_zero": (c_i32, [vp, c_i64, vp]),
    "dsvg_gemm_group_scope": (c_i32, [c_i32, vp]),
    "dsvg_colsum": (c_i32, [c_i32, vp, c_i64, c_i64, c_i32, vp, c_i32, c_f32, c_u32, vp, vp, c_i64, vp]),
    "dsvg_colsum_workspace_bytes": (c_i64, [c_i64, c_i32]),
    "dsvg_layernorm_fwd": (c_i32, [c_i32, vp, vp, vp, vp, vp, vp, c_i64, c_i32, c_f32, vp]),
    "dsvg_layernorm_bwd": (c_i32, [c_i32, vp, vp, vp, vp, vp, vp, vp, vp, vp, c_i32, c_i64, c_i32, vp, c_i64, vp]),
    "dsvg_layernorm_bwd_workspace_bytes": (c_i64, [c_i64, c_i32]),
    "dsvg_layernorm_bwd_masked": (c_i32, [c_i32, vp, vp, vp, vp, vp, vp, vp, vp, vp, c_i32, c_i64, c_i32, vp, c_i64, vp, c_f32,
                                          c_u32, vp, vp]),
    "dsvg_attention_fwd": (c_i32, [c_i32, vp, vp, vp, c_i64, vp, vp, c_i64, c_i32, c_i32, c_f32, c_f32, c_u32, vp, vp]),
    "dsvg_attention_bwd": (c_i32, [c_i32, vp, vp, vp, c_i64, vp, vp, vp, c_i64, c_i32, c_i32, c_f32, c_f32, c_u32, vp, vp]),
    "dsvg_attention_tiles": (c_i32, [vp, c_i64, c_i32, vp, vp, vp]),
    "dsvg_pack_tokens": (c_i32, [vp, vp, vp, c_i64, c_i32, c_i32, vp, vp, vp, vp, vp]),
    "dsvg_visible_first": (c_i32, [vp, c_i64, vp, vp, vp, vp]),
    "dsvg_head_pack_elems": (c_i64, [c_i32]),
    "dsvg_head_pack": (c_i32, [vp, c_i32, vp, vp]),
    "dsvg_head_argmax": (c_i32, [vp, vp, vp, c_i64, c_i32, c_i32, vp, vp]),
    "dsvg_head_sample": (c_i32, [vp, vp, vp, c_i64, c_i32, c_i32, c_f32, vp, c_u32, vp, vp]),
    "dsvg_head_lse_workspace_bytes": (c_i64, [c_i64]),
    "dsvg_head_lse": (c_i32, [vp, vp, vp, c_i64, c_i32, c_i32, vp, vp, vp, vp, vp, vp, c_i64, vp]),
    "dsvg_head_dlogits": (c_i32, [vp, vp, vp, c_i64, c_i32, c_i32, vp, vp, vp, vp, vp, vp, c_f32, vp, c_i64, vp]),
    "dsvg_attention_bwd_outproj": (c_i32, [vp, vp, vp, c_i64, vp, vp, vp, vp, c_i64, c_i32, c_f32, c_f32, c_u32, vp, vp]),
    "dsvg_attn_pack_bwd_elems": (c_i64, [c_i32]),
    "dsvg_attn_pack_bwd": (c_i32, [vp, vp, c_i32, vp, vp]),
    "dsvg_ffn_wgrad_finish_many": (c_i32, [vp, c_i32, vp]),
    "dsvg_ffn_debug_clock": (c_i32, [vp]),
    "dsvg_gs_debug_clock": (c_i32, [vp]),
    "dsvg_gather_groups": (c_i32, [c_i32, vp, vp, vp, c_i64, c_i32, c_i32, c_i64, vp]),
    "dsvg_build_masks": (c_i32, [vp, c_i64, c_i32, c_i32, c_i32, vp, vp, vp, vp]),
    "dsvg_embed_gather": (c_i32, [c_i32, vp, vp, vp, vp, vp, vp, vp, vp, c_i64, c_i32, c_i32, c_i32, c_i32, c_i32, vp]),
    "dsvg_embed_scatter": (c_i32, [c_i32, vp, vp, vp, vp, vp, vp, vp, vp, c_i64, c_i32, c_i32, c_i32, c_i32, c_i32,
                                   c_i32, vp, c_i64, vp]),
    "dsvg_embed_scatter_workspace_bytes": (c_i64, [c_i64, c_i32, c_i32, c_i32, c_i32, c_i32, c_i32]),
    "dsvg_group_index": (c_i32, [vp, c_i64, c_i32, c_i32, vp, vp]),
    "dsvg_add_pos_fwd": (c_i32, [c_i32, vp, vp, vp, c_i64, c_i32, c_i32, c_f32, c_u32, vp, vp]),
    "dsvg_add_pos_bwd": (c_i32, [c_i32, vp, vp, vp, c_i32, c_i64, c_i32, c_i32, c_f32, c_u32, vp, vp, c_i64, vp]),
    "dsvg_add_pos_bwd_workspace_bytes": (c_i64, [c_i64, c_i32, c_i32]),
    "dsvg_masked_mean_fwd": (c_i32, [c_i32, vp, vp, vp, vp, c_i64, c_i32, c_i32, vp]),
    "dsvg_masked_mean_bwd": (c_i32, [c_i32, vp, vp, vp, c_i64, vp, c_i64, c_i32, c_i32, vp]),
    "dsvg_bcast_add_fwd": (c_i32, [c_i32, vp, vp, c_i64, c_i32, c_i32, c_f32, c_u32, vp, vp]),
    "dsvg_bcast_add_bwd": (c_i32, [c_i32, vp, vp, c_i64, c_i64, c_i32, c_i32, c_f32, c_u32, vp, c_i64, vp]),
    "dsvg_bcast_add_bwd_masked": (c_i32, [vp, vp, vp, c_i64, c_i64, c_i32, c_i32, c_i64, c_f32, c_u32, c_u32, vp, c_i64, vp]),
    "dsvg_loss_targets": (c_i32, [vp, vp, vp, c_i64, c_i32, c_i32, c_i32, c_i32, vp, vp, vp, vp, vp, vp, vp]),
    "dsvg_masked_ce_fwd": (c_i32, [c_i32, vp, c_i64, c_i32, vp, vp, c_i64, c_i32, vp, vp, vp, c_i64, vp, vp]),
    "dsvg_masked_ce_workspace_bytes": (c_i64, [c_i64]),
    "dsvg_masked_ce_bwd": (c_i32, [c_i32, vp, c_i64, c_i32, vp, vp, vp, vp, vp, c_f32, vp, c_i64, c_i64, c_i32, vp, c_i32, vp]),
    "dsvg_live_rows": (c_i32, [vp, c_i64, c_i32, vp, vp, vp, c_i64, vp]),
    "dsvg_live_rows_workspace_bytes": (c_i64, [c_i64]),
    "dsvg_scatter_rows": (c_i32, [c_i32, vp, vp, vp, c_i64, c_i32, c_i32, vp]),
    "dsvg_sumsq": (c_i32, [vp, c_i64, vp, vp, c_i64, vp]),
    "dsvg_sumsq_workspace_bytes": (c_i64, [c_i64]),
    "dsvg_adamw_step": (c_i32, [vp, vp, vp, vp, c_i64, vp, c_f32, c_f32, c_f32, c_f32, vp, vp, c_f32, c_f32, vp]),
    "dsvg_cast_weights": (c_i32, [c_i32, vp, vp, vp, c_i64, c_i64, vp]),
    "dsvg_advance_step": (c_i32, [vp, vp, vp]),
    "dsvg_pack_images": (c_i32, [vp, vp, c_i64, vp, c_i32, vp, vp, vp, vp, vp, c_i32, vp, vp, vp, c_i32, vp, vp, vp, vp, vp]),
    "dsvg_copy_many": (c_i32, [vp, vp, vp, c_i32, vp]),
    "dsvg_loss_combine_fwd": (c_i32, [vp, vp, c_i32, vp, vp]),
    "dsvg_loss_combine_bwd": (c_i32, [vp, vp, vp, c_i32, vp, vp]),
    "dsvg_gate_mul": (c_i32, [c_i32, vp, vp, vp, c_i64, c_f32, vp]),
    "dsvg_add": (c_i32, [c_i32, vp, vp, vp, c_i64, vp]),
    "dsvg_drop_apply": (c_i32, [c_i32, vp, vp, c_i64, c_f32, c_u32, vp, vp]),
    "dsvg_assemble_batch": (c_i32, [vp, c_i64, vp, c_i64, vp, c_i64, c_i32, c_i32, c_i32, c_f32, c_i32, vp, vp, vp,
                                    vp]),
    "dsvg_attention_causal_fwd": (c_i32, [c_i32, vp, vp, vp, c_i64, c_i32, c_i32, c_f32, c_f32, c_u32, vp, vp]),
    "dsvg_attention_causal_bwd": (c_i32, [c_i32, vp, vp, vp, vp, c_i64, c_i32, c_i32, c_f32, c_f32, c_u32, vp, vp]),
    "dsvg_seq_lens": (c_i32, [vp, c_i64, c_i32, c_i32, vp, vp]),
    "dsvg_attention_long_fwd": (c_i32, [c_i32, vp, vp, vp, c_i64, c_i32, c_i32, c_f32, c_i32, c_i32, c_f32, c_u32, vp,
                                        vp]),
    "dsvg_attention_long_bwd": (c_i32, [c_i32, vp, vp, vp, vp, c_i64, c_i32, c_i32, c_f32, c_i32, c_f32, c_u32, vp, vp]),
    "dsvg_prefix_mean_fwd": (c_i32, [c_i32, vp, vp, vp, c_i64, c_i32, c_i32, vp]),
    "dsvg_prefix_mean_bwd": (c_i32, [c_i32, vp, vp, vp, c_i64, c_i32, c_i32, vp]),
    "dsvg_build_masks_lens": (c_i32, [vp, c_i64, c_i32, c_i32, c_i32, vp, vp, vp, vp]),
    "dsvg_pack_tokens_lens": (c_i32, [vp, vp, vp, c_i64, c_i32, c_i32, vp, vp, vp, vp, vp]),
    "dsvg_packed_mean_fwd": (c_i32, [c_i32, vp, vp, vp, c_i64, c_i32, vp]),
    "dsvg_packed_mean_bwd": (c_i32, [c_i32, vp, vp, c_i64, vp, c_i64, c_i32, vp]),
    "dsvg_attention_long_packed_fwd": (c_i32, [c_i32, vp, vp, c_i64, vp, c_i64, c_i32, c_i32, c_f32, c_f32, c_u32, vp,
                                               vp]),
    "dsvg_attention_long_packed_bwd": (c_i32, [c_i32, vp, vp, c_i64, vp, vp, c_i64, c_i32, c_i32, c_f32, c_f32, c_u32,
                                               vp, vp]),
    "dsvg_attention_long_mfma_fwd": (c_i32, [vp, vp, vp, c_i64, vp, c_i64, c_i32, c_i32, c_f32, c_f32, c_u32, vp, vp]),
    "dsvg_attention_long_mfma_bwd": (c_i32, [vp, vp, vp, c_i64, vp, vp, c_i64, c_i32, c_i32, c_f32, c_f32, c_u32, vp,
                                             vp]),
    "dsvg_match_costs": (c_i32, [c_i32, vp, c_i64, vp, c_i64, vp, c_i64, vp, vp, vp, c_i64, c_i32, c_i32, c_i32, c_i32,
                                 c_i32, c_i32, c_i32, c_f32, c_f32, c_f32, vp, vp, vp]),
    "dsvg_match_assign": (c_i32, [vp, vp, c_i64, c_i32, c_i32, vp, vp, vp, vp]),
    "dsvg_argmax_rows": (c_i32, [c_i32, vp, c_i64, c_i32, c_i64, c_i32, vp, vp]),
    "dsvg_sample_rows": (c_i32, [c_i32, vp, c_i64, c_i32, c_i64, c_i32, c_f32, vp, c_u32, vp, vp]),
    "dsvg_sample_points": (c_i32, [c_i32, vp, vp, c_i64, c_i32, c_i32, c_i32, vp, vp, vp]),
    "dsvg_chamfer_workspace_bytes": (c_i64, [c_i64, c_i64, c_i64]),
    "dsvg_chamfer": (c_i32, [vp, vp, c_i64, vp, vp, c_i64, c_i64, vp, vp, c_i64, vp]),
    "dsvg_chamfer_nn": (c_i32, [vp, vp, c_i64, vp, vp, c_i64, c_i64, vp, vp, vp, vp, c_i64, vp]),
    "dsvg_chamfer_bwd": (c_i32, [vp, vp, c_i64, vp, vp, c_i64, c_i64, vp, vp, vp, vp, vp, vp]),
    "dsvg_sample_points_bwd": (c_i32, [vp, c_i64, c_i32, c_i32, c_i32, vp, vp, vp]),
    "dsvg_emd_workspace_bytes": (c_i64, [c_i64, c_i64]),
    "dsvg_emd": (c_i32, [vp, vp, c_i64, vp, vp, c_i64, c_i64, c_i32, vp, vp, vp, vp, vp, c_i64, vp]),
    "dsvg_emd_bwd": (c_i32, [vp, vp, c_i64, vp, vp, vp, vp, c_i32, c_i64, vp, vp]),
    "dsvg_polyline_length": (c_i32, [vp, vp, c_i64, c_i64, vp, vp]),
    "dsvg_polyline_length_bwd": (c_i32, [vp, vp, c_i64, c_i64, vp, vp, vp]),
    "dsvg_raster_workspace_bytes": (c_i64, [c_i64, c_i32, c_i32, c_i32, c_i32]),
    "dsvg_raster_segments": (c_i32, [c_i32, vp, vp, c_i64, c_i32, c_i32, c_i32, c_i32, vp, c_i64, vp, vp]),
    "dsvg_raster_sweep": (c_i32, [vp, vp, c_i64, c_i64, c_i32, c_f32, c_i32, vp, vp]),
    "dsvg_raster_sweep_nn": (c_i32, [vp, vp, c_i64, c_i64, c_i32, c_f32, c_i32, vp, vp, vp]),
    "dsvg_raster_sweep_bwd": (c_i32, [vp, vp, vp, vp, vp, c_i64, c_i64, c_i32, c_f32, c_i32, vp, vp]),
    "dsvg_raster_segments_bwd": (c_i32, [vp, vp, vp, c_i64, c_i32, c_i32, c_i32, c_i32, vp, vp]),
    "dsvg_ffn_pack_bytes": (c_i64, [c_i32, c_i32]),
    "dsvg_ffn_pack": (c_i32, [vp, vp, c_i32, c_i32, c_i32, vp, vp, vp, vp, vp]),
    "dsvg_ffn_fwd": (c_i32, [vp, vp, vp, vp, vp, vp, vp, vp, c_i64, c_f32, c_f32, c_u32, c_u32, vp, c_i32, vp]),
    "dsvg_ffn_bwd_dx": (c_i32, [vp, vp, vp, vp, vp, c_i64, c_f32, vp, c_f32, c_u32, vp, vp]),
    "dsvg_ffn_gate_dw2": (c_i32, [vp, vp, vp, c_f32, vp, c_i64, c_i32, vp, vp, vp, c_i64, vp]),
    "dsvg_ffn_wgrad_finish": (c_i32, [vp] * 12),
    "dsvg_probe_trread": (c_i32, [vp, vp, vp]),
    "dsvg_attn_pack_bytes": (c_i64, [c_i32]),
    "dsvg_attn_pack": (c_i32, [vp, vp, c_i32, c_i32, c_i32, vp, vp]),
    "dsvg_attn_block_fwd": (c_i32, [vp, vp, vp, vp, vp, vp, vp, vp, vp, c_i64, c_i32, c_i64, vp, vp, vp, vp, vp, vp,
                                    c_f32, c_f32, c_f32, c_u32, c_u32, vp, vp, c_i64, c_u32, vp]),
    "dsvg_gs_pack_bytes": (c_i64, [c_i32]),
    "dsvg_gs_pack": (c_i32, [vp, vp, c_i32, c_i32, c_i32, c_i32, vp, vp, vp]),
    "dsvg_gs_layer_fwd": (c_i32, [vp] * 12 + [c_i64, c_i64, c_i32] + [vp] * 11 + [c_f32, c_f32, c_f32, c_u32, vp, c_i64, c_i32, vp]),
    "dsvg_gs_bwd_workspace_bytes": (c_i64, [c_i64, c_i32]),
    "dsvg_latent_chain_fwd": (c_i32, [vp, vp, vp, c_i32, vp, vp, vp, c_i64, vp]),
    "dsvg_latent_chain_bwd": (c_i32, [vp, vp, vp, c_i32, vp, vp, c_i64, vp]),
    "dsvg_gs_layer_bwd": (c_i32, [vp] * 13 + [c_i64, c_i32] + [vp] * 10 + [c_f32, c_f32, c_u32, vp, vp, c_i64, vp, vp]),
    "dsvg_gs_stack_fwd": (c_i32, [vp, vp, c_i32, vp, c_i64, c_i64, c_i32, c_f32, c_f32, c_f32, vp, vp]),
    "dsvg_gs_stack_bwd": (c_i32, [vp, vp, c_i32, vp, c_i64, c_i32, c_f32, c_f32, vp, c_i64, c_i64, vp]),
}

_lib = None


class DsvgError(RuntimeError):
    pass


def load():
    global _lib
    if _lib is not None:
        return _lib
    if not os.path.exists(LIB_PATH):
        raise DsvgError(
            f"{LIB_PATH} not found: the HIP extension is not built. Run `python -c \"import __graft_entry__ as g; "
            f"g.build()\"` (needs hipcc); there is no CPU fallback for the product path.")
    lib = C.CDLL(LIB_PATH)
    for name, (res, args) in SIGNATURES.items():
        fn = getattr(lib, name)
        fn.restype = res
        fn.argtypes = args
    built = lib.dsvg_version()
    if built != ABI_VERSION:
        raise DsvgError(f"{LIB_PATH} was built with DSVG_ABI_VERSION {built}, this binding expects {ABI_VERSION}: rebuild "
                        f"the library (deepsvg_amd/csrc/build.sh)")
    _lib = lib
    return lib


def check(rc, what):
    if rc != 0:
        msg = load().dsvg_last_error()
        raise DsvgError(f"{what} failed (rc={rc}): {msg.decode() if msg else '?'}")
```

deepsvg_amd/ops.py:

```python
import ctypes as C
import os

import torch

from . import lib as _l

F32, BF16 = _l.DSVG_F32, _l.DSVG_BF16
RELU = 1

PROFILE_ON = False
PROFILE = []
PROFILE_KEEP_DEFER = False
_TAG = None


def _event():
    return torch.cuda.Event(enable_timing=True)


class tag:

    def __init__(self, name):
        self.name = name

# ... 235 lines not shown
        _rowmajor(gate)
        assert gate.dtype == a.dtype and tuple(gate.shape) == (M, N)
        d.ldgate, d.gate_scale = gate.stride(0), float(gate_scale)
    d.drop_p, d.drop_site = float(drop_p), int(drop_site)
    d.a_drop_p, d.a_drop_site, d.a_drop_ld = float(a_drop_p), int(a_drop_site), a.shape[1]
    if drop_p > 0 or a_drop_p > 0:
        assert seed is not None and seed.dtype == torch.int64
    d.accumulate = int(accumulate)
    d.impl = impl
    ws_bytes = 0
    if split_k > 1:
        assert odt == torch.float32 and (out is None or out.is_contiguous())
        ws_bytes = _l.load().dsvg_gemm_workspace_bytes(M, N, split_k)
        d.split_k = split_k
        if rowsum is not None:
            assert rowsum.dtype == torch.float32 and rowsum.is_contiguous() and rowsum.numel() == M
    else:
        assert rowsum is None, "rowsum needs split_k > 1"
    return d, M, N, odt, ws_bytes


def gemm(a, b, *, a_kc=True, b_kc=True, bias=None, res=None, res_pre=False, act=0, gate=None, gate_scale=1.0,
         drop_p=0.0, drop_site=0, a_drop_p=0.0, a_drop_site=0, seed=None, out=None, out_dtype=None,
         accumulate=False, split_k=1, impl=0, rowsum=None):
    _chk(a, b, bias, res, gate, seed, out)
    key = (a.dtype, a.shape, a.stride(0), b.shape, b.stride(0), a_kc, b_kc, bias is not None,
           None if res is None else (res.shape, res.stride(0)), res_pre, act,
           None if gate is None else (gate.shape, gate.stride(0)), gate_scale, drop_p, drop_site, a_drop_p,
           a_drop_site, out_dtype if out is None else (out.dtype, out.shape, out.stride(0), out.stride(1)),
           accumulate, split_k, impl, rowsum is not None)
    ent = _GEMM_CACHE.get(key)
    if ent is None:
        ent = _gemm_build(a, b, a_kc, b_kc, bias, res, res_pre, act, gate, gate_scale, drop_p, drop_site, a_drop_p,
                          a_drop_site, seed, out, out_dtype, accumulate, split_k, impl, rowsum)
        if len(_GEMM_CACHE) < 4096:
            _GEMM_CACHE[key] = ent
    d, M, N, odt, ws_bytes = ent
    if out is None:
        out = torch.empty((M, N), dtype=odt, device=a.device)
    d.A, d.B, d.C = a.data_ptr(), b.data_ptr(), out.data_ptr()
    d.bias = bias.data_ptr() if bias is not None else None
    d.res = res.data_ptr() if res is not None else None
    d.gate = gate.data_ptr() if gate is not None else None
    d.seed = seed.data_ptr() if (seed is not None and (drop_p > 0 or a_drop_p > 0)) else None
    d.rowsum = rowsum.data_ptr() if rowsum is not None else None
    ws = None
    if ws_bytes:
        ws = _ws(ws_bytes, a.device)
        d.workspace, d.workspace_bytes = ws.data_ptr(), ws.numel() * 4
    L = _l.load()
    if PROFILE_ON and _TAG is not None:
        esz = 2 if a.dtype == torch.bfloat16 else 4
        extra = (esz * d.M * d.N if (res is not None or gate is not None) else 0)
        if _GroupScope.active is not None and split_k > 1 and not a_kc and not b_kc:
            _l.check(L.dsvg_gemm(C.byref(d), _stream()), "dsvg_gemm")
            m = _GroupScope.active.setdefault(_TAG, [0.0, 0.0])
            m[0] += 2.0 * d.M * d.N * d.K
            m[1] += float(esz * (d.M * d.K + d.N * d.K) + out.element_size() * d.M * d.N)
            return out
        ev0, ev1 = _event(), _event()
        ev0.record()
        _l.check(L.dsvg_gemm(C.byref(d), _stream()), "dsvg_gemm")
        ev1.record()
        spec = dict(a=tuple(a.shape), b=tuple(b.shape), a_kc=a_kc, b_kc=b_kc, bias=bias is not None, res=res is not None,
                    act=act, gate=gate is not None, gate_scale=gate_scale, drop_p=drop_p, split_k=split_k,
                    rowsum=rowsum is not None, out_f32=out.dtype == torch.float32, dtype=str(a.dtype))
        PROFILE.append((_TAG, ev0, ev1, 2.0 * d.M * d.N * d.K,
                        float(esz * (d.M * d.K + d.N * d.K) + out.element_size() * d.M * d.N + extra), spec))
        return out
    _l.check(L.dsvg_gemm(C.byref(d), _stream()), "dsvg_gemm")
    return out


_SPLITK_BLOCKS = int(os.environ.get("DSVG_SPLITK_BLOCKS", "256"))
_SPLITK_REFILL = int(os.environ.get("DSVG_SPLITK_REFILL", "480"))


def split_k_for(M, N, K, target_blocks=None):
    default_target = target_blocks is None
    target_blocks = target_blocks or _SPLITK_BLOCKS
    tiles = ((M + 127) // 128) * ((N + 127) // 128)
    s = max(1, target_blocks // tiles)
    s = min(s, max(1, K // 128))
    if s >= 8:
        s = s // 8 * 8
        if default_target and _SPLITK_REFILL > 0 and K >= 16384 and tiles * s < 0.8 * target_blocks:
            s2 = min((_SPLITK_REFILL // tiles) // 8 * 8, max(1, K // 128) // 8 * 8)
            if s2 > s:
                s = s2
    return s


def colsum(a, *, out=None, accumulate=False, drop_p=0.0, drop_site=0, seed=None):
    _chk(a, out, seed)
    _rowmajor(a)
    M, N = a.shape
    if out is None:
        out = torch.empty(N, dtype=torch.float32, device=a.device)
    assert out.dtype == torch.float32 and out.is_contiguous() and out.numel() == N
    L = _l.load()
    ws = _ws(L.dsvg_colsum_workspace_bytes(M, N), a.device)
    _l.check(L.dsvg_colsum(_dt(a), a.data_ptr(), a.stride(0), M, N, out.data_ptr(), int(accumulate), float(drop_p),
                           int(drop_site), _p(seed) if drop_p > 0 else None, ws.data_ptr(), ws.numel() * 4,
                           _stream()), "dsvg_colsum")
    return out


def layernorm_fwd(x, gamma, beta, eps=1e-5):
    _chk(x, gamma, beta)
    assert x.is_contiguous() and x.dim() == 2
    rows, d = x.shape
    y = torch.empty_like(x)
    mean = torch.empty(rows, dtype=torch.float32, device=x.device)
    rstd = torch.empty(rows, dtype=torch.float32, device=x.device)
    ev = _prof_begin()
    _l.check(_l.load().dsvg_layernorm_fwd(_dt(x), x.data_ptr(), gamma.data_ptr(), beta.data_ptr(), y.data_ptr(),
                                          mean.data_ptr(), rstd.data_ptr(), rows, d, float(eps), _stream()),
             "dsvg_layernorm_fwd")
    _prof_end(ev, 0.0, 0.0, dict(op="layernorm_fwd"))
    return y, mean, rstd


def layernorm_bwd(dy, x, mean, rstd, gamma, *, res=None, dgamma=None, dbeta=None, accumulate=False, dx=None, masked=None):
    _chk(dy, x, mean, rstd, gamma, res, dgamma, dbeta)
    assert dy.is_contiguous() and x.is_contiguous() and dy.shape == x.shape
    rows, d = x.shape
    if dx is None:
        dx = torch.empty_like(x)
    if dgamma is None:
        dgamma = torch.empty(d, dtype=torch.float32, device=x.device)
    if dbeta is None:
        dbeta = torch.empty(d, dtype=torch.float32, device=x.device)
    if res is not None:
        assert res.is_contiguous() and res.shape == x.shape and res.dtype == x.dtype
    L = _l.load()
    ws = _ws(L.dsvg_layernorm_bwd_workspace_bytes(rows, d), x.device)
    ev = _prof_begin()
    if masked is not None:
        mp, msite, mseed = masked
        dxm = torch.empty_like(dx)
        _l.check(L.dsvg_layernorm_bwd_masked(_dt(x), dy.data_ptr(), x.data_ptr(), mean.data_ptr(), rstd.data_ptr(),
                                             gamma.data_ptr(), _p(res), dx.data_ptr(), dgamma.data_ptr(), dbeta.data_ptr(),
                                             int(accumulate), rows, d, ws.data_ptr(), ws.numel() * 4, dxm.data_ptr(),
                                             float(mp), int(msite), _p(mseed) if mp > 0 else None, _stream()),
                 "dsvg_layernorm_bwd_masked")
        _prof_end(ev, 0.0, 0.0, dict(op="layernorm_bwd"))
        return dx, dgamma, dbeta, dxm
    _l.check(L.dsvg_layernorm_bwd(_dt(x), dy.data_ptr(), x.data_ptr(), mean.data_ptr(), rstd.data_ptr(),
                                  gamma.data_ptr(), _p(res), dx.data_ptr(), dgamma.data_ptr(), dbeta.data_ptr(),
                                  int(accumulate), rows, d, ws.data_ptr(), ws.numel() * 4, _stream()),
             "dsvg_layernorm_bwd")
    _prof_end(ev, 0.0, 0.0, dict(op="layernorm_bwd"))
    return dx, dgamma, dbeta


def attention_tiles(seq_off, n_seq, max_rows=32):
    _chk(seq_off)
    assert seq_off.dtype == torch.int32 and seq_off.numel() == n_seq + 1
    tiles = torch.empty(n_seq + 2, dtype=torch.int32, device=seq_off.device)
    scratch = torch.empty((n_seq + 63) // 64 * 64, dtype=torch.int32, device=seq_off.device)
    _l.check(_l.load().dsvg_attention_tiles(seq_off.data_ptr(), n_seq, max_rows, tiles.data_ptr(), scratch.data_ptr(),
                                            _stream()), "dsvg_attention_tiles")
    return tiles


LONG_MFMA = os.environ.get("DSVG_LONG_MFMA", "1") != "0"


def _long_route(qkv, S, causal, seq_off, path_stage):
    if S <= 64 or causal or not (path_stage or seq_off is not None):
        return None
    return "mfma" if (qkv.dtype == torch.bfloat16 and LONG_MFMA) else ("packed" if seq_off is not None else "padded")


def attention_fwd(qkv, key_mask, n_seq, S, n_heads, scale, drop_p=0.0, drop_site=0, seed=None, seq_off=None,
                  tiles=None, causal=False, only_row=None, out=None, path_stage=False):
    _chk(qkv, key_mask, seed, seq_off)
    rows = qkv.shape[0]
    assert qkv.is_contiguous() and qkv.shape[1] == 3 * 32 * n_heads, "attention needs head_dim == 32"
    assert (rows >= n_seq * S) if seq_off is None else (key_mask is None and seq_off.numel() == n_seq + 1)
    if out is None:
        out = torch.empty((rows, 32 * n_heads), dtype=qkv.dtype, device=qkv.device)
    route = _long_route(qkv, S, causal, seq_off, path_stage)
    if route is not None:
        assert key_mask is None or key_mask.dtype == torch.int32
        sd = _p(seed) if drop_p > 0 else None
        if route == "mfma":
            _l.check(_l.load().dsvg_attention_long_mfma_fwd(qkv.data_ptr(), _p(key_mask), _p(seq_off), rows, out.data_ptr(),
                                                            n_seq, S, n_heads, float(scale), float(drop_p), int(drop_site),
                                                            sd, _stream()), "dsvg_attention_long_mfma_fwd")
            if seq_off is None:
                out[n_seq * S:].zero_()
        elif route == "padded":
            _l.check(_l.load().dsvg_attention_long_fwd(_dt(qkv), qkv.data_ptr(), _p(key_mask), out.data_ptr(), n_seq, S,
                                                       n_heads, float(scale), 0, -1, float(drop_p), int(drop_site), sd,
                                                       _stream()), "dsvg_attention_long_fwd")
            out[n_seq * S:].zero_()
        else:
            _l.check(_l.load().dsvg_attention_long_packed_fwd(_dt(qkv), qkv.data_ptr(), seq_off.data_ptr(), rows,
                                                              out.data_ptr(), n_seq, S, n_heads, float(scale), float(drop_p),
                                                              int(drop_site), sd, _stream()),
                     "dsvg_attention_long_packed_fwd")
        return out
    if S > 64:
        assert seq_off is None and rows == n_seq * S and (key_mask is None or key_mask.dtype == torch.int32)
        _l.check(_l.load().dsvg_attention_long_fwd(_dt(qkv), qkv.data_ptr(), _p(key_mask), out.data_ptr(), n_seq, S,
                                                   n_heads, float(scale), 1 if causal else 0,
                                                   -1 if only_row is None else int(only_row), float(drop_p),
                                                   int(drop_site), _p(seed) if drop_p > 0 else None, _stream()),
                 "dsvg_attention_long_fwd")
        return out
    if causal:
        assert seq_off is None and rows == n_seq * S
        _l.check(_l.load().dsvg_attention_causal_fwd(_dt(qkv), qkv.data_ptr(), _p(key_mask), out.data_ptr(), n_seq, S,
                                                     n_heads, float(scale), float(drop_p), int(drop_site),
                                                     _p(seed) if drop_p > 0 else None, _stream()),
                 "dsvg_attention_causal_fwd")
        return out
    _l.check(_l.load().dsvg_attention_fwd(_dt(qkv), qkv.data_ptr(), _p(key_mask), _p(seq_off), rows, _p(tiles),
                                          out.data_ptr(), n_seq, S, n_heads, float(scale), float(drop_p), int(drop_site),
                                          _p(seed) if drop_p > 0 else None, _stream()), "dsvg_attention_fwd")
    return out


def attention_bwd(qkv, key_mask, dout, n_seq, S, n_heads, scale, drop_p=0.0, drop_site=0, seed=None, seq_off=None,
                  tiles=None, causal=False, path_stage=False):
    _chk(qkv, key_mask, dout, seed, seq_off)
    assert qkv.is_contiguous() and dout.is_contiguous() and dout.dtype == qkv.dtype
    assert seq_off is None or (key_mask is None and seq_off.numel() == n_seq + 1)
    dqkv = torch.empty_like(qkv)
    route = _long_route(qkv, S, causal, seq_off, path_stage)
    if route is not None:
        assert key_mask is None or key_mask.dtype == torch.int32
        assert seq_off is not None or qkv.shape[0] >= n_seq * S
        sd = _p(seed) if drop_p > 0 else None
        if route == "mfma":
            _l.check(_l.load().dsvg_attention_long_mfma_bwd(qkv.data_ptr(), _p(key_mask), _p(seq_off), qkv.shape[0],
                                                            dout.data_ptr(), dqkv.data_ptr(), n_seq, S, n_heads,
                                                            float(scale), float(drop_p), int(drop_site), sd, _stream()),
                     "dsvg_attention_long_mfma_bwd")
            if seq_off is None:
                dqkv[n_seq * S:].zero_()
        elif route == "padded":
            _l.check(_l.load().dsvg_attention_long_bwd(_dt(qkv), qkv.data_ptr(), _p(key_mask), dout.data_ptr(),
                                                       dqkv.data_ptr(), n_seq, S, n_heads, float(scale), 0, float(drop_p),
                                                       int(drop_site), sd, _stream()), "dsvg_attention_long_bwd")
            dqkv[n_seq * S:].zero_()
        else:
            _l.check(_l.load().dsvg_attention_long_packed_bwd(_dt(qkv), qkv.data_ptr(), seq_off.data_ptr(), qkv.shape[0],
                                                              dout.data_ptr(), dqkv.data_ptr(), n_seq, S, n_heads,
                                                              float(scale), float(drop_p), int(drop_site), sd, _stream()),
                     "dsvg_attention_long_packed_bwd")
        return dqkv
    if S > 64:
        assert seq_off is None and qkv.shape[0] == n_seq * S and (key_mask is None or key_mask.dtype == torch.int32)
        _l.check(_l.load().dsvg_attention_long_bwd(_dt(qkv), qkv.data_ptr(), _p(key_mask), dout.data_ptr(),
                                                   dqkv.data_ptr(), n_seq, S, n_heads, float(scale), 1 if causal else 0,
                                                   float(drop_p), int(drop_site), _p(seed) if drop_p > 0 else None,
                                                   _stream()), "dsvg_attention_long_bwd")
        return dqkv
    if causal:
        assert seq_off is None and qkv.shape[0] == n_seq * S
        _l.check(_l.load().dsvg_attention_causal_bwd(_dt(qkv), qkv.data_ptr(), _p(key_mask), dout.data_ptr(),
                                                     dqkv.data_ptr(), n_seq, S, n_heads, float(scale), float(drop_p),
                                                     int(drop_site), _p(seed) if drop_p > 0 else None, _stream()),
                 "dsvg_attention_causal_bwd")
        return dqkv
    _l.check(_l.load().dsvg_attention_bwd(_dt(qkv), qkv.data_ptr(), _p(key_mask), _p(seq_off), qkv.shape[0],
                                          _p(tiles), dout.data_ptr(), dqkv.data_ptr(), n_seq, S, n_heads, float(scale),
                                          float(drop_p), int(drop_site), _p(seed) if drop_p > 0 else None, _stream()),
             "dsvg_attention_bwd")
    return dqkv


ATTN_BWD_LAYER_ELEMS = 128 * 512


def attn_pack_bwd(flat, offs, n_layers, packed=None):
    _chk(flat, offs, packed)
    assert flat.dtype == torch.float32 and offs.dtype == torch.int64 and offs.is_contiguous() and tuple(offs.shape) == (n_layers, 2)
    if packed is None:
        packed = torch.empty(n_layers * ATTN_BWD_LAYER_ELEMS, dtype=torch.bfloat16, device=flat.device)
    assert packed.numel() == n_layers * ATTN_BWD_LAYER_ELEMS and packed.dtype == torch.bfloat16
    _l.check(_l.load().dsvg_attn_pack_bwd(flat.data_ptr(), offs.data_ptr(), n_layers, packed.data_ptr(), _stream()),
             "dsvg_attn_pack_bwd")
    return packed


def attention_bwd_outproj(qkv, key_mask, dx1m, wo_packed_bwd, n_seq, S, scale, drop_p=0.0, drop_site=0, seed=None, seq_off=None,
                          tiles=None):
    _chk(qkv, key_mask, dx1m, wo_packed_bwd, seed, seq_off, tiles)
    assert qkv.dtype == torch.bfloat16 and qkv.is_contiguous() and qkv.shape[1] == 768
    assert dx1m.dtype == qkv.dtype and dx1m.is_contiguous() and tuple(dx1m.shape) == (qkv.shape[0], 256)
    assert wo_packed_bwd.numel() == ATTN_BWD_LAYER_ELEMS and wo_packed_bwd.is_contiguous()
    assert (seq_off is None) == (tiles is None) and (seq_off is None or (key_mask is None and seq_off.numel() == n_seq + 1))
    dqkv = torch.empty_like(qkv)
    _l.check(_l.load().dsvg_attention_bwd_outproj(qkv.data_ptr(), _p(key_mask), _p(seq_off), qkv.shape[0], _p(tiles),
                                                  dx1m.data_ptr(), wo_packed_bwd.data_ptr(), dqkv.data_ptr(), n_seq, S,
                                                  float(scale), float(drop_p), int(drop_site),
                                                  _p(seed) if drop_p > 0 else None, _stream()),
             "dsvg_attention_bwd_outproj")
    return dqkv


def seq_lens(commands, S, eos_id=4):
    _chk(commands)
# ... 1263 lines not shown
```

include/dsvg.h:

```cpp
#ifndef DSVG_H
#define DSVG_H

#include <stdint.h>
#include <stddef.h>

#ifdef __cplusplus
extern "C" {
#endif

#define DSVG_F32 0
#define DSVG_BF16 1
#define DSVG_I64 2

#define DSVG_ABI_VERSION 18

const char* dsvg_last_error(void);
int dsvg_version(void);

typedef struct dsvg_gemm_desc {
    int32_t dtype;
    int32_t M, N, K;
    const void* A; int64_t lda; int32_t a_kc;
    const void* B; int64_t ldb; int32_t b_kc;
    void* C; int64_t ldc; int32_t c_f32;
    const float* bias;
    const void* res; int64_t ldres; int32_t res_pre;
    int32_t act;
    const void* gate; int64_t ldgate; float gate_scale;
    float drop_p; uint32_t drop_site;
    float a_drop_p; uint32_t a_drop_site; int64_t a_drop_ld;
    const uint64_t* seed;
    int32_t accumulate;
    int32_t split_k; float* workspace; int64_t workspace_bytes;
    float* rowsum;
    int32_t impl;
} dsvg_gemm_desc;

int dsvg_gemm(const dsvg_gemm_desc* d, void* stream);
int64_t dsvg_gemm_workspace_bytes(int32_t M, int32_t N, int32_t split_k);

int dsvg_reduce_partials(const float* partial, int64_t P, int64_t n, float* out, int32_t accumulate,
                         void* stream);

int dsvg_defer_scope(int32_t on, void* stream);
int dsvg_defer_zero(float* out, int64_t n, void* stream);
int dsvg_flush_deferred(void* stream);
int dsvg_gemm_group_scope(int32_t on, void* stream);

int dsvg_colsum(int32_t dtype, const void* A, int64_t lda, int64_t M, int32_t N, float* out,
                int32_t accumulate, float drop_p, uint32_t drop_site, const uint64_t* seed,
                float* workspace, int64_t workspace_bytes, void* stream);
int64_t dsvg_colsum_workspace_bytes(int64_t M, int32_t N);

int dsvg_layernorm_fwd(int32_t dtype, const void* x, const float* gamma, const float* beta, void* y,
                       float* mean, float* rstd, int64_t rows, int32_t d, float eps, void* stream);
int dsvg_layernorm_bwd(int32_t dtype, const void* dy, const void* x, const float* mean,
                       const float* rstd, const float* gamma, const void* res, void* dx,
                       float* dgamma, float* dbeta, int32_t accumulate, int64_t rows, int32_t d,
                       float* workspace, int64_t workspace_bytes, void* stream);
int64_t dsvg_layernorm_bwd_workspace_bytes(int64_t rows, int32_t d);
int dsvg_layernorm_bwd_masked(int32_t dtype, const void* dy, const void* x, const float* mean, const float* rstd,
                              const float* gamma, const void* res, void* dx, float* dgamma, float* dbeta,
                              int32_t accumulate, int64_t rows, int32_t d, float* workspace, int64_t workspace_bytes,
                              void* dx_masked, float drop_p, uint32_t drop_site, const void* seed, void* stream);

int dsvg_attention_fwd(int32_t dtype, const void* qkv, const uint64_t* key_mask, const int32_t* seq_off,
                       int64_t total_rows, const int32_t* tile_first, void* out, int64_t n_seq, int32_t S,
                       int32_t n_heads, float scale, float drop_p, uint32_t drop_site, const uint64_t* seed,
                       void* stream);
int dsvg_attention_bwd(int32_t dtype, const void* qkv, const uint64_t* key_mask, const int32_t* seq_off,
                       int64_t total_rows, const int32_t* tile_first, const void* dout, void* dqkv, int64_t n_seq,
                       int32_t S, int32_t n_heads, float scale, float drop_p, uint32_t drop_site,
                       const uint64_t* seed, void* stream);
int dsvg_attention_tiles(const int32_t* seq_off, int64_t n_seq, int32_t max_rows, int32_t* tile_first,
                         int32_t* scratch, void* stream);

int dsvg_build_masks(const float* commands, int64_t n_seq, int32_t S, int32_t G, int32_t eos_id,
                     uint64_t* key_mask, int32_t* seq_visible, uint64_t* group_mask, void* stream);

int dsvg_embed_gather(int32_t dtype, const float* commands, const float* args,
                      const float* command_embed, const float* arg_embed, const float* group_embed,
                      const int32_t* groups, void* A, void* R, int64_t T, int32_t n_args, int32_t E,
                      int32_t d, int32_t n_cmd, int32_t n_argvals, void* stream);
int dsvg_embed_scatter(int32_t dtype, const float* commands, const float* args,
                       const int32_t* groups, const void* dA, const void* dR, float* d_arg_embed,
                       float* d_command_embed, float* d_group_embed, int64_t T, int32_t n_args,
                       int32_t E, int32_t d, int32_t n_cmd, int32_t n_argvals, int32_t n_groups,
                       float* workspace, int64_t workspace_bytes, void* stream);
int64_t dsvg_embed_scatter_workspace_bytes(int64_t T, int32_t n_args, int32_t E, int32_t d,
                                           int32_t n_cmd, int32_t n_argvals, int32_t n_groups);
int dsvg_group_index(const float* commands, int64_t n_seq, int32_t S, int32_t m_id, int32_t* groups,
                     void* stream);
int dsvg_visible_first(const int32_t* visible, int64_t n, int32_t* new_of_old, int32_t* old_of_new,
                       int32_t* n_visible, void* stream);
int dsvg_gather_groups(int32_t dtype, const void* src, const int32_t* idx, void* dst, int64_t n_groups,
                       int32_t S, int32_t width, int64_t n_src, void* stream);
int dsvg_pack_tokens(const float* commands, const float* args, const uint64_t* key_mask, int64_t n_seq,
                     int32_t S, int32_t n_args, int32_t* seq_off, float* packed_commands,
                     float* packed_args, int32_t* packed_pos, void* stream);

int dsvg_add_pos_fwd(int32_t dtype, const void* x, const float* pos, void* y, int64_t n_seq, int32_t S,
                     int32_t d, float drop_p, uint32_t drop_site, const uint64_t* seed, void* stream);
int dsvg_add_pos_bwd(int32_t dtype, const void* dy, void* dx, float* d_pos, int32_t accumulate,
                     int64_t n_seq, int32_t S, int32_t d, float drop_p, uint32_t drop_site,
                     const uint64_t* seed, float* workspace, int64_t workspace_bytes, void* stream);
int64_t dsvg_add_pos_bwd_workspace_bytes(int64_t n_seq, int32_t S, int32_t d);

int dsvg_masked_mean_fwd(int32_t dtype, const void* x, const uint64_t* mask, const int32_t* seq_off,
                         void* out, int64_t n_seq, int32_t S, int32_t d, void* stream);
int dsvg_masked_mean_bwd(int32_t dtype, const void* dout, const uint64_t* mask, const int32_t* seq_off,
                         int64_t total_rows, void* dx, int64_t n_seq, int32_t S, int32_t d, void* stream);

int dsvg_bcast_add_fwd(int32_t dtype, void* x, const void* g, int64_t n_seq, int32_t S, int32_t d,
                       float drop_p, uint32_t drop_site, const uint64_t* seed, void* stream);
int dsvg_bcast_add_bwd(int32_t dtype, const void* dx, void* dg, int64_t n_seq, int64_t n_seq_out, int32_t S, int32_t d,
                       float drop_p, uint32_t drop_site, const uint64_t* seed, int64_t dg_ld, void* stream);
int dsvg_bcast_add_bwd_masked(const void* dx, void* dg, void* dx_masked, int64_t n_seq, int64_t n_seq_out, int32_t S, int32_t d,
                              int64_t rows, float drop_p, uint32_t drop_site, uint32_t mask_site, const uint64_t* seed,
                              int64_t dg_ld, void* stream);

int dsvg_loss_targets(const float* tgt_commands, const float* tgt_args, const float* cmd_args_mask,
                      int64_t n_seq, int32_t S1, int32_t n_args, int32_t n_cmd, int32_t eos_id,
                      int32_t* cmd_tgt, float* cmd_w, int32_t* arg_tgt, float* arg_w, int32_t* vis_tgt,
                      const int32_t* seq_perm, void* stream);
int dsvg_masked_ce_fwd(int32_t dtype, const void* logits, int64_t ld, int32_t group, const int32_t* target,
                       const float* w, int64_t rows, int32_t C, float* lse, float* sum_count,
                       float* workspace, int64_t workspace_bytes, const int32_t* tok_idx, void* stream);
int64_t dsvg_masked_ce_workspace_bytes(int64_t rows);
int dsvg_masked_ce_bwd(int32_t dtype, const void* logits, int64_t ld, int32_t group, const int32_t* target,
                       const float* w, const float* lse, const float* sum_count, const float* gscale,
                       float coef, void* dlogits, int64_t ld_d, int64_t rows, int32_t C,
                       const int32_t* tok_idx, int32_t logits_compact, void* stream);
int dsvg_loss_combine_fwd(const float* const* sum_count, const float* weights, int32_t n, float* out, void* stream);
int dsvg_loss_combine_bwd(const float* dtotal, const float* const* dterms, const float* weights, int32_t n,
                          float* dsum_count, void* stream);
int dsvg_live_rows(const float* w, int64_t n_tok, int32_t group, int32_t* live, int32_t* count,
                   int32_t* workspace, int64_t workspace_bytes, void* stream);
int64_t dsvg_live_rows_workspace_bytes(int64_t n_tok);
int dsvg_scatter_rows(int32_t dtype, const void* src, const int32_t* idx, void* dst, int64_t n_rows,
                      int32_t width, int32_t accumulate, void* stream);

int dsvg_sumsq(const float* x, int64_t n, float* out , float* workspace, int64_t workspace_bytes,
               void* stream);
int64_t dsvg_sumsq_workspace_bytes(int64_t n);
int dsvg_adamw_step(float* p, const float* g, float* m, float* v, int64_t n, const float* lr,
                    float beta1, float beta2, float eps, float weight_decay, const int64_t* step,
                    const float* gnorm_sq, float max_norm, float grad_scale, void* stream);
int dsvg_cast_weights(int32_t dtype, const float* src, void* dst, void* dst_t, int64_t rows,
                      int64_t cols, void* stream);
int dsvg_advance_step(int64_t* counter, uint64_t* seed, void* stream);
int dsvg_pack_images(const float* flat_f32, void* flat_bf16, int64_t n,
                     const int64_t* ffn_offs, int32_t ffn_layers, void* ffn_fwd, void* ffn_bwd, float* ffn_b1f, void* ffn_w2p,
                     const int64_t* attn_offs, int32_t attn_layers, void* attn_img, void* attn_bwd,
                     const int64_t* gs_offs, int32_t gs_layers, void* gs_fwd, void* gs_bwd,
                     int64_t* counter, uint64_t* seed, void* stream);
int dsvg_copy_many(const void* const* src, void* const* dst, const int64_t* bytes, int32_t n, void* stream);
int dsvg_gate_mul(int32_t dtype, const void* dy, const void* y, void* out, int64_t n, float scale, void* stream);
int dsvg_drop_apply(int32_t dtype, const void* x, void* y, int64_t n, float drop_p, uint32_t drop_site,
                    const uint64_t* seed, void* stream);
int dsvg_add(int32_t dtype, const void* a, const void* b, void* out, int64_t n, void* stream);
int dsvg_attention_causal_fwd(int32_t dtype, const void* qkv, const uint64_t* key_mask, void* out, int64_t n_seq,
                              int32_t S, int32_t n_heads, float scale, float drop_p, uint32_t drop_site,
                              const uint64_t* seed, void* stream);
int dsvg_attention_bwd_outproj(const void* qkv, const uint64_t* key_mask, const int32_t* seq_off, int64_t total_rows,
                               const int32_t* tile_first, const void* dx1m, const void* wo_packed_bwd, void* dqkv,
                               int64_t n_seq, int32_t S, float scale, float drop_p, uint32_t drop_site,
                               const uint64_t* seed, void* stream);
int64_t dsvg_attn_pack_bwd_elems(int32_t n_layers);
int dsvg_attn_pack_bwd(const float* flat_f32, const int64_t* offs, int32_t n_layers, void* packed_bwd, void* stream);
int dsvg_attention_causal_bwd(int32_t dtype, const void* qkv, const uint64_t* key_mask, const void* dout, void* dqkv,
                              int64_t n_seq, int32_t S, int32_t n_heads, float scale, float drop_p,
                              uint32_t drop_site, const uint64_t* seed, void* stream);

int dsvg_seq_lens(const float* commands, int64_t n_seq, int32_t S, int32_t eos_id, int32_t* lens, void* stream);
int dsvg_attention_long_fwd(int32_t dtype, const void* qkv, const int32_t* seq_len, void* out, int64_t n_seq, int32_t S,
                            int32_t n_heads, float scale, int32_t causal, int32_t only_row, float drop_p,
                            uint32_t drop_site, const uint64_t* seed, void* stream);
int dsvg_attention_long_bwd(int32_t dtype, const void* qkv, const int32_t* seq_len, const void* dout, void* dqkv,
                            int64_t n_seq, int32_t S, int32_t n_heads, float scale, int32_t causal, float drop_p,
                            uint32_t drop_site, const uint64_t* seed, void* stream);
int dsvg_prefix_mean_fwd(int32_t dtype, const void* x, const int32_t* lens, void* out, int64_t n_seq, int32_t S, int32_t d,
                         void* stream);
int dsvg_prefix_mean_bwd(int32_t dtype, const void* dout, const int32_t* lens, void* dx, int64_t n_seq, int32_t S,
                         int32_t d, void* stream);

int dsvg_build_masks_lens(const float* commands, int64_t n_seq, int32_t S, int32_t G, int32_t eos_id, int32_t* lens,
                          int32_t* seq_visible, uint64_t* group_mask, void* stream);
int dsvg_pack_tokens_lens(const float* commands, const float* args, const int32_t* lens, int64_t n_seq, int32_t S,
                          int32_t n_args, int32_t* seq_off, float* packed_commands, float* packed_args,
                          int32_t* packed_pos, void* stream);
int dsvg_packed_mean_fwd(int32_t dtype, const void* x, const int32_t* seq_off, void* out, int64_t n_seq, int32_t d,
                         void* stream);
int dsvg_packed_mean_bwd(int32_t dtype, const void* dout, const int32_t* seq_off, int64_t total_rows, void* dx,
                         int64_t n_seq, int32_t d, void* stream);
int dsvg_attention_long_packed_fwd(int32_t dtype, const void* qkv, const int32_t* seq_off, int64_t total_rows, void* out,
                                   int64_t n_seq, int32_t S, int32_t n_heads, float scale, float drop_p,
                                   uint32_t drop_site, const uint64_t* seed, void* stream);
int dsvg_attention_long_packed_bwd(int32_t dtype, const void* qkv, const int32_t* seq_off, int64_t total_rows,
                                   const void* dout, void* dqkv, int64_t n_seq, int32_t S, int32_t n_heads, float scale,
                                   float drop_p, uint32_t drop_site, const uint64_t* seed, void* stream);
int dsvg_attention_long_mfma_fwd(const void* qkv, const int32_t* lens, const int32_t* seq_off, int64_t total_rows,
                                 void* out, int64_t n_seq, int32_t S, int32_t n_heads, float scale, float drop_p,
                                 uint32_t drop_site, const uint64_t* seed, void* stream);
int dsvg_attention_long_mfma_bwd(const void* qkv, const int32_t* lens, const int32_t* seq_off, int64_t total_rows,
                                 const void* dout, void* dqkv, int64_t n_seq, int32_t S, int32_t n_heads, float scale,
                                 float drop_p, uint32_t drop_site, const uint64_t* seed, void* stream);

int dsvg_match_costs(int32_t dtype, const void* cmd_logits, int64_t ld_c, const void* args_logits, int64_t ld_a,
                     const void* vis_logits, int64_t ld_v, const float* tgt_commands, const float* tgt_args,
                     const float* cmd_args_mask, int64_t N, int32_t G, int32_t Gp, int32_t S1, int32_t n_args,
                     int32_t args_dim, int32_t n_cmd, int32_t eos_id, float w_args, float w_cmd, float w_vis,
                     float* cost, int32_t* visible, void* stream);
int dsvg_match_assign(const float* cost, const int32_t* visible, int64_t N, int32_t G, int32_t Gp,
                      int32_t* assign, int32_t* idx, int32_t* inv, void* stream);

int dsvg_argmax_rows(int32_t dtype, const void* logits, int64_t ld, int32_t group, int64_t rows, int32_t C,
                     int32_t* out, void* stream);
// ... 149 lines not shown
```

Baseline: 93220 icons/s.

## Co-schedule attention input-projection weight-grad GEMM with LayerNorm backward in one launch

Adds a horizontally fused kernel whose workgroups take on either the split-K weight-gradient GEMM role (dqkv^T x xn1) or the LayerNorm backward role. The LN role reuses the GEMM role's static LDS, and the dispatch order between the two roles is configurable. The LN backward body is factored into a shared header so it can handle two row blocks per workgroup, and the split-K reduction is pulled out into a reusable helper. The aim is to fill the GPU with two independent, individually under-occupying kernels at once and save a launch. In exchange, each role's occupancy is bound by the other's LDS and register needs, and the GEMM weight-grad can no longer overlap in the way it did before.

```diff
diff --git a/deepsvg_amd/csrc/gemm.hip b/deepsvg_amd/csrc/gemm.hip
--- a/deepsvg_amd/csrc/gemm.hip
+++ b/deepsvg_amd/csrc/gemm.hip
@@ -725,6 +725,25 @@
 int dsvg_gemm_bf16_launch(const dsvg_gemm_desc& d, int k_chunk, int nsplit, float* part, float* rs_part,
                           hipStream_t st, int* part_is_bf16);
 
+int dsvg_gemm_splitk_reduce(const dsvg_gemm_desc& d, int nsplit, float* part, float* rs_part, int part_bf16, hipStream_t st) {
+    const size_t slice = dsvg_splitk_slice(d.M, d.N, d.rowsum != nullptr);
+    const int64_t mn = (int64_t)d.M * d.N;
+    if (part_bf16) {
+        if (rs_part && d.rowsum == (float*)d.C + mn && !(d.M & 3))
+            return dsvg_reduce_partials_mixed(part, nsplit, (int64_t)slice, mn + d.M, mn, (float*)d.C, d.accumulate, st);
+        int rc = dsvg_reduce_partials_mixed(part, nsplit, (int64_t)slice, mn, mn, (float*)d.C, d.accumulate, st);
+        if (rc) return rc;
+        if (rs_part) return dsvg_reduce_partials_strided(rs_part, nsplit, (int64_t)slice, d.M, d.rowsum, d.accumulate, st);
+        return 0;
+    }
+    if (rs_part && d.rowsum == (float*)d.C + mn)
+        return dsvg_reduce_partials_strided(part, nsplit, (int64_t)slice, mn + d.M, (float*)d.C, d.accumulate, st);
+    int rc = dsvg_reduce_partials_strided(part, nsplit, (int64_t)slice, mn, (float*)d.C, d.accumulate, st);
+    if (rc) return rc;
+    if (rs_part) return dsvg_reduce_partials_strided(rs_part, nsplit, (int64_t)slice, d.M, d.rowsum, d.accumulate, st);
+    return 0;
+}
+
 extern "C" int dsvg_gemm(const dsvg_gemm_desc* dp, void* stream) {
     DSVG_CHECK_ARG(dp, "gemm: null desc");
     dsvg_gemm_desc d = *dp;
@@ -798,22 +817,6 @@
         int rc = dsvg_gemm_bf16_launch(d, k_chunk, nsplit, part, rs_part, st, &part_bf16);
         if (rc) return rc;
     }
-    if (part && part_bf16) {
-        const int64_t mn = (int64_t)d.M * d.N;
-        if (rs_part && d.rowsum == (float*)d.C + mn && !(d.M & 3))
-            return dsvg_reduce_partials_mixed(part, nsplit, (int64_t)slice, mn + d.M, mn, (float*)d.C, d.accumulate, st);
-        int rc = dsvg_reduce_partials_mixed(part, nsplit, (int64_t)slice, mn, mn, (float*)d.C, d.accumulate, st);
-        if (rc) return rc;
-        if (rs_part) return dsvg_reduce_partials_strided(rs_part, nsplit, (int64_t)slice, d.M, d.rowsum, d.accumulate, st);
-        return 0;
-    }
-    if (part) {
-        const int64_t mn = (int64_t)d.M * d.N;
-        if (rs_part && d.rowsum == (float*)d.C + mn)
-            return dsvg_reduce_partials_strided(part, nsplit, (int64_t)slice, mn + d.M, (float*)d.C, d.accumulate, st);
-        int rc = dsvg_reduce_partials_strided(part, nsplit, (int64_t)slice, mn, (float*)d.C, d.accumulate, st);
-        if (rc) return rc;
-        if (rs_part) return dsvg_reduce_partials_strided(rs_part, nsplit, (int64_t)slice, d.M, d.rowsum, d.accumulate, st);
-    }
+    if (part) return dsvg_gemm_splitk_reduce(d, nsplit, part, rs_part, part_bf16, st);
     return 0;
 }
diff --git a/deepsvg_amd/csrc/gemm_bf16.h b/deepsvg_amd/csrc/gemm_bf16.h
--- a/deepsvg_amd/csrc/gemm_bf16.h
+++ b/deepsvg_amd/csrc/gemm_bf16.h
@@ -14,3 +14,4 @@
 bool dsvg_gemm_bf16_glds_try(const dsvg_gemm_desc& d, int epi, dim3 grid, int tiles_n, int nwg, int k_chunk,
                              float* part, float* rs_part, int mode, hipStream_t st, int* part_is_bf16);
 int dsvg_gemm_group_flush(hipStream_t st);
+int dsvg_gemm_splitk_reduce(const dsvg_gemm_desc& d, int nsplit, float* part, float* rs_part, int part_bf16, hipStream_t st);
diff --git a/deepsvg_amd/csrc/gemm_bf16_glds.hip b/deepsvg_amd/csrc/gemm_bf16_glds.hip
--- a/deepsvg_amd/csrc/gemm_bf16_glds.hip
+++ b/deepsvg_amd/csrc/gemm_bf16_glds.hip
@@ -1,4 +1,5 @@
 #include "gemm_bf16.h"
+#include "ln_bwd_body.h"
 #include "mfma_frag.h"
 #include <map>
 #include <mutex>
@@ -44,12 +45,17 @@
         : "memory", "scc");
 }
 
+template <int NST>
+__device__ __forceinline__ bf16_t* glds_static_smem() {
+    __shared__ __attribute__((aligned(1024))) bf16_t smem_static[NST <= 2 ? NST * 2 * IMG : 8];
+    return smem_static;
+}
+
 template <bool AKC, bool BKC, int EPI, int NST>
 __device__ __forceinline__ void glds_body(const dsvg_gemm_desc& p, int tiles_n, int nwg_mn, int k_chunk, float* part,
                                           float* rs_part, int mode, int part_bf16, int bid, int bid_y) {
-    __shared__ __attribute__((aligned(1024))) bf16_t smem_static[NST <= 2 ? NST * 2 * IMG : 8];
     extern __shared__ __attribute__((aligned(1024))) bf16_t smem_dynamic[];
-    bf16_t* const smem = NST <= 2 ? smem_static : smem_dynamic;
+    bf16_t* const smem = NST <= 2 ? glds_static_smem<NST>() : smem_dynamic;
 
     const int xcd = bid % 8, local = bid / 8;
     int wgid, kz;
@@ -412,6 +418,50 @@
     glds_body<false, false, EPI_PARTIAL, 4>(p, w.tiles_n, w.nwg_mn, w.k_chunk, w.part, w.rs_part, w.mode, w.part_bf16,
                                             local % w.grid_x, local / w.grid_x);
 }
+
+struct WgLnArgs {
+    const bf16_t* dy; const bf16_t* x; const float* mean; const float* rstd; const float* gamma; const bf16_t* res;
+    bf16_t* dx; float* part; bf16_t* dxm; const uint64_t* seed;
+    long long rows;
+    float drop_p; uint32_t site;
+    int nb, n_phys;
+    int runs_gemm, runs;
+    int order;
+};
+
+template <int NVB>
+__global__ __launch_bounds__(256, 4) void gemm_wgrad_ln_bwd_kernel(const WgItem w, const WgLnArgs a) {
+    const int run = (int)blockIdx.x >> 3, x8 = (int)blockIdx.x & 7;
+    int gemm_run, ln_run;
+    if (a.order == 0) {
+        const int before = (int)((long long)run * a.runs_gemm / a.runs);
+        const bool is_gemm = (int)((long long)(run + 1) * a.runs_gemm / a.runs) > before;
+        gemm_run = is_gemm ? before : -1;
+        ln_run = is_gemm ? -1 : run - before;
+    } else if (a.order == 1) {
+        gemm_run = run < a.runs_gemm ? run : -1;
+        ln_run = run - a.runs_gemm;
+    } else {
+        const int runs_ln = a.runs - a.runs_gemm;
+        ln_run = run < runs_ln ? run : -1;
+        gemm_run = run - runs_ln;
+    }
+    if (gemm_run >= 0) {
+        const int local = gemm_run * 8 + x8;
+        if (local >= w.first_block) return;
+        dsvg_gemm_desc p;
+        p.A = w.A; p.B = w.B; p.M = w.M; p.N = w.N; p.K = w.K; p.lda = w.lda; p.ldb = w.ldb;
+        glds_body<false, false, EPI_PARTIAL, 1>(p, w.tiles_n, w.nwg_mn, w.k_chunk, w.part, w.rs_part, w.mode, w.part_bf16,
+                                                local % w.grid_x, local / w.grid_x);
+        return;
+    }
+    const int j = ln_run * 8 + x8;
+    if (j >= a.n_phys) return;
+    ln_bwd_body<bf16_t, 1, NVB>(a.dy, a.x, a.mean, a.rstd, a.gamma, a.res, a.dx, a.part, a.rows, 256, a.dxm, a.drop_p, a.seed,
+                                a.site, reinterpret_cast<float*>(glds_static_smem<1>()), (unsigned)j, (unsigned)a.nb,
+                                (unsigned)a.n_phys);
+}
+static_assert(2 * ln_bwd_lds_floats(256) * sizeof(float) <= 2 * IMG * sizeof(bf16_t), "the LayerNorm role lives in the GEMM role's LDS");
 
 struct GroupQueue {
     int scope = 0;
@@ -565,3 +615,66 @@
     }
     return rc;
 }
+
+extern "C" int dsvg_gemm_wgrad_ln_bwd(const dsvg_gemm_desc* gp, int32_t dtype, const void* dy, const void* x, const float* mean,
+                                      const float* rstd, const float* gamma, const void* res, void* dx, float* dgamma,
+                                      float* dbeta, int32_t accumulate, int64_t rows, int32_t d, float* workspace,
+                                      int64_t workspace_bytes, void* dx_masked, float drop_p, uint32_t drop_site,
+                                      const void* seed, void* stream) {
+    DSVG_CHECK_ARG(gp, "gemm_wgrad_ln_bwd: null desc");
+    const dsvg_gemm_desc g = *gp;
+    hipStream_t st = (hipStream_t)stream;
+    DSVG_CHECK_ARG(g.dtype == DSVG_BF16 && dtype == DSVG_BF16, "gemm_wgrad_ln_bwd: bf16 only");
+    DSVG_CHECK_ARG(g.A && g.B && g.C && g.M > 0 && g.N > 0 && g.K > 0, "gemm_wgrad_ln_bwd: bad GEMM operands");
+    DSVG_CHECK_ARG(!g.a_kc && !g.b_kc, "gemm_wgrad_ln_bwd: both GEMM operands must be token-major");
+    DSVG_CHECK_ARG(g.split_k > 1, "gemm_wgrad_ln_bwd: needs split_k > 1");
+    DSVG_CHECK_ARG((g.K % GBK) == 0, "gemm_wgrad_ln_bwd: K = %d is no multiple of %d", g.K, GBK);
+    DSVG_CHECK_ARG(g.c_f32 && g.ldc == g.N && !g.bias && !g.res && !g.gate && g.act == 0 && !(g.drop_p > 0.f) &&
+                   !(g.a_drop_p > 0.f), "gemm_wgrad_ln_bwd: split-K needs a dense fp32 C and no prologue / epilogue");
+    DSVG_CHECK_ARG(g.workspace && g.workspace_bytes >= dsvg_gemm_workspace_bytes(g.M, g.N, g.split_k),
+                   "gemm_wgrad_ln_bwd: split_k workspace too small");
+    DSVG_CHECK_ARG(!(g.lda & 7) && !(g.ldb & 7) && !((uintptr_t)g.A & 15) && !((uintptr_t)g.B & 15) && g.M >= 8 &&
+                   !(g.N & 7) && g.lda >= ((g.M + 7) / 8) * 8 && g.ldb >= g.N && !((uintptr_t)g.workspace & 15),
+                   "gemm_wgrad_ln_bwd: GEMM operands miss the LDS-DMA kernel's alignment rules");
+    DSVG_CHECK_ARG(((size_t)GBK * g.lda + g.M) * 2 < (1ull << 32) && ((size_t)GBK * g.ldb + g.N) * 2 < (1ull << 32),
+                   "gemm_wgrad_ln_bwd: GEMM operand rows too long for 32-bit byte offsets");
+    const int k_chunk = ((g.K + g.split_k - 1) / g.split_k + 63) / 64 * 64;
+    int nsplit = (g.K + k_chunk - 1) / k_chunk;
+    if ((g.split_k % 8) == 0) nsplit = g.split_k;
+    static const bool force_2d = getenv("DSVG_SPLITK_2D") != nullptr;
+    static const bool pbf_on = !(getenv("DSVG_SPLITK_BF16") && atoi(getenv("DSVG_SPLITK_BF16")) == 0);
+    float* part = g.workspace;
+    float* rs_part = g.rowsum ? part + (size_t)g.M * g.N : nullptr;
+    WgItem w;
+    w.A = g.A; w.B = g.B; w.part = part; w.rs_part = rs_part;
+    w.M = g.M; w.N = g.N; w.K = g.K; w.lda = g.lda; w.ldb = g.ldb;
+    w.tiles_n = dsvg_cdiv(g.N, GBN);
+    w.nwg_mn = dsvg_cdiv(g.M, GBM) * w.tiles_n;
+    w.k_chunk = k_chunk;
+    w.mode = (nsplit > 1 && (nsplit % 8) == 0 && !force_2d) ? 1 : 0;
+    w.grid_x = w.mode == 1 ? w.nwg_mn * nsplit : w.nwg_mn;
+    w.first_block = w.nwg_mn * nsplit;
+    w.part_bf16 = pbf_on ? 1 : 0;
+    DSVG_CHECK_ARG(dy && x && mean && rstd && gamma && dx && dgamma && dbeta, "gemm_wgrad_ln_bwd: null LayerNorm pointer");
+    DSVG_CHECK_ARG(rows > 0 && d == 256, "gemm_wgrad_ln_bwd: LayerNorm needs rows > 0 and d = 256");
+    DSVG_CHECK_ARG(workspace && workspace_bytes >= dsvg_layernorm_bwd_workspace_bytes(rows, d),
+                   "gemm_wgrad_ln_bwd: LayerNorm workspace too small");
+    DSVG_CHECK_ARG(dx_masked != dx, "gemm_wgrad_ln_bwd: the masked output needs a buffer of its own");
+    DSVG_CHECK_ARG(!(dx_masked && drop_p > 0.f) || seed, "gemm_wgrad_ln_bwd: dropout needs a seed");
+    static const int nvb = getenv("DSVG_WGRAD_LN_NVB") ? atoi(getenv("DSVG_WGRAD_LN_NVB")) : 2;
+    static const int order = getenv("DSVG_WGRAD_LN_ORDER") ? atoi(getenv("DSVG_WGRAD_LN_ORDER")) : 2;
+    WgLnArgs a;
+    a.dy = (const bf16_t*)dy; a.x = (const bf16_t*)x; a.mean = mean; a.rstd = rstd; a.gamma = gamma; a.res = (const bf16_t*)res;
+    a.dx = (bf16_t*)dx; a.part = workspace; a.dxm = (bf16_t*)dx_masked; a.seed = (const uint64_t*)seed;
+    a.rows = (long long)rows; a.drop_p = drop_p; a.site = drop_site;
+    a.nb = dsvg_ln_bwd_grid(rows);
+    a.n_phys = nvb == 1 ? a.nb : dsvg_cdiv(a.nb, 2);
+    a.runs_gemm = dsvg_cdiv(w.first_block, 8);
+    a.runs = a.runs_gemm + dsvg_cdiv(a.n_phys, 8);
+    a.order = order;
+    if (nvb == 1) hipLaunchKernelGGL(gemm_wgrad_ln_bwd_kernel<1>, dim3(8 * a.runs), dim3(256), 0, st, w, a);
+    else hipLaunchKernelGGL(gemm_wgrad_ln_bwd_kernel<2>, dim3(8 * a.runs), dim3(256), 0, st, w, a);
+    DSVG_LAUNCH_CHECK("gemm_wgrad_ln_bwd");
+    if (int rc = dsvg_gemm_splitk_reduce(g, nsplit, part, rs_part, w.part_bf16, st)) return rc;
+    return dsvg_ln_bwd_reduce(workspace, a.nb, d, dgamma, dbeta, accumulate, st);
+}
diff --git a/deepsvg_amd/csrc/layernorm.hip b/deepsvg_amd/csrc/layernorm.hip
--- a/deepsvg_amd/csrc/layernorm.hip
+++ b/deepsvg_amd/csrc/layernorm.hip
@@ -1,8 +1,7 @@
 #include "dsvg_common.h"
+#include "ln_bwd_body.h"
 #include "../../include/dsvg.h"
 
-constexpr int LN_MAXV_MAX = 4;
-constexpr int LN_MAX_BLOCKS = 1024;
 
 template <typename T, int LN_MAXV>
 __global__ __launch_bounds__(256) void ln_fwd_kernel(const T* __restrict__ x, const float* __restrict__ gamma,
@@ -71,113 +70,12 @@
                                                      T* dx, float* __restrict__ part,
                                                      long long rows, int d, T* dxm, float drop_p,
                                                      const uint64_t* __restrict__ seed, uint32_t site) {
-    const DropCtx dmc = drop_make(dxm ? drop_p : 0.f, seed, site);
     extern __shared__ float red_raw[];
-    const int nvec = d / 4 + 1;
-    auto red = [&](int w, int k, int vec, int e) -> float& { return red_raw[((w * 2 + k) * nvec + vec) * 4 + e]; };
-    const int lane = threadIdx.x & 63;
-    const int wave = threadIdx.x >> 6;
-    const int nv = d / 256 + ((d % 256) ? 1 : 0);
-    float ag[LN_MAXV][4], ab[LN_MAXV][4];
-#pragma unroll
-    for (int i = 0; i < LN_MAXV; ++i)
-#pragma unroll
-        for (int e = 0; e < 4; ++e) { ag[i][e] = 0.f; ab[i][e] = 0.f; }
-
-    float4 g4[LN_MAXV];
-#pragma unroll
-    for (int i = 0; i < LN_MAXV; ++i) g4[i] = *reinterpret_cast<const float4*>(gamma + min(i * 256 + lane * 4, d - 4));
-    for (long long row = (long long)blockIdx.x * 4 + wave; row < rows; row += (long long)gridDim.x * 4) {
-        const float mu = mean[row], rs = rstd[row];
-        float xh[LN_MAXV][4], gd[LN_MAXV][4], rv[LN_MAXV][4];
-        float c1 = 0.f, c2 = 0.f;
-#pragma unroll
-        for (int i = 0; i < LN_MAXV; ++i) {
-            const int c = i * 256 + lane * 4;
-            if (i < nv && c < d) {
-                float xv[4], dv[4];
-                Elem<T>::ld4(x + row * d + c, xv);
-                Elem<T>::ld4(dy + row * d + c, dv);
-                if (res) Elem<T>::ld4(res + row * d + c, rv[i]);
-                const float4 g = g4[i];
-                const float gg[4] = {g.x, g.y, g.z, g.w};
-#pragma unroll
-                for (int e = 0; e < 4; ++e) {
-                    xh[i][e] = (xv[e] - mu) * rs;
-                    gd[i][e] = gg[e] * dv[e];
-                    c1 += gd[i][e];
-                    c2 += gd[i][e] * xh[i][e];
-                    ag[i][e] += dv[e] * xh[i][e];
-                    ab[i][e] += dv[e];
-                }
-            } else {
-#pragma unroll
-                for (int e = 0; e < 4; ++e) { xh[i][e] = 0.f; gd[i][e] = 0.f; }
-            }
-        }
-        c1 = wave_sum(c1) / (float)d;
-        c2 = wave_sum(c2) / (float)d;
-#pragma unroll
-        for (int i = 0; i < LN_MAXV; ++i) {
-            const int c = i * 256 + lane * 4;
-            if (i < nv && c < d) {
-                float o[4];
-#pragma unroll
-                for (int e = 0; e < 4; ++e) o[e] = rs * (gd[i][e] - c1 - xh[i][e] * c2);
-                if (res) {
-#pragma unroll
-                    for (int e = 0; e < 4; ++e) o[e] += rv[i][e];
-                }
-                Elem<T>::st4(dx + row * d + c, o);
-                if (dxm) {
-                    const uint64_t id4 = (uint64_t)row * (uint64_t)d + (uint64_t)c;
-                    float mm[4] = {1.f, 1.f, 1.f, 1.f};
-                    if (dmc.on) {
-                        const uint32_t hg = drop_group(dmc, id4 >> 3);
-                        const uint32_t wb = ((uint32_t)id4 & 4u) ? 2u : 0u;
-                        const uint32_t w0 = drop_word(hg, wb), w1 = drop_word(hg, wb + 1u);
-                        mm[0] = (w0 & 0xffffu) < dmc.thresh ? 0.f : dmc.scale;
-                        mm[1] = (w0 >> 16) < dmc.thresh ? 0.f : dmc.scale;
-                        mm[2] = (w1 & 0xffffu) < dmc.thresh ? 0.f : dmc.scale;
-                        mm[3] = (w1 >> 16) < dmc.thresh ? 0.f : dmc.scale;
-                    }
-                    float om[4];
-#pragma unroll
-                    for (int e = 0; e < 4; ++e) {
-                        T t;
-                        Elem<T>::st(&t, o[e]);
-                        om[e] = Elem<T>::ld(&t) * mm[e];
-                    }
-                    Elem<T>::st4(dxm + row * d + c, om);
-                }
-            }
-        }
-    }
-#pragma unroll
-    for (int i = 0; i < LN_MAXV; ++i) {
-        if (i < nv) {
-#pragma unroll
-            for (int e = 0; e < 4; ++e) {
-                if (i * 256 + lane * 4 < d) {
-                    red(wave, 0, i * 64 + lane, e) = ag[i][e];
-                    red(wave, 1, i * 64 + lane, e) = ab[i][e];
-                }
-            }
-        }
-    }
-    __syncthreads();
-    float* pg = part + (size_t)blockIdx.x * 2 * d;
-    for (int c = threadIdx.x; c < d; c += 256) {
-        const int vec = c >> 2, e = c & 3;
-        float sg = 0.f, sb = 0.f;
-#pragma unroll
-        for (int w = 0; w < 4; ++w) { sg += red(w, 0, vec, e); sb += red(w, 1, vec, e); }
-        pg[c] = sg;
-        pg[d + c] = sb;
-    }
+    ln_bwd_body<T, LN_MAXV, 1>(dy, x, mean, rstd, gamma, res, dx, part, rows, d, dxm, drop_p, seed, site, red_raw,
+                               blockIdx.x, gridDim.x, 0u);
 }
 
-static int ln_grid(long long rows) {
+int dsvg_ln_bwd_grid(long long rows) {
     static const int cap = getenv("DSVG_LN_BLOCKS") ? atoi(getenv("DSVG_LN_BLOCKS")) : LN_MAX_BLOCKS;
     long long nb = (rows + 3) / 4;
     return (int)(nb < cap ? nb : cap);
@@ -204,7 +102,7 @@
 }
 
 extern "C" int64_t dsvg_layernorm_bwd_workspace_bytes(int64_t rows, int32_t d) {
-    return (int64_t)ln_grid(rows) * 2 * d * (int64_t)sizeof(float);
+    return (int64_t)dsvg_ln_bwd_grid(rows) * 2 * d * (int64_t)sizeof(float);
 }
 
 static int ln_bwd_launch(int32_t dtype, const void* dy, const void* x, const float* mean, const float* rstd,
@@ -242,8 +140,8 @@
     DSVG_CHECK_ARG(workspace && workspace_bytes >= dsvg_layernorm_bwd_workspace_bytes(rows, d),
                    "layernorm_bwd: workspace too small");
     hipStream_t st = (hipStream_t)stream;
-    const int nb = ln_grid(rows);
-    const size_t lds = (size_t)4 * 2 * (d / 4 + 1) * 4 * sizeof(float);
+    const int nb = dsvg_ln_bwd_grid(rows);
+    const size_t lds = ln_bwd_lds_floats(d) * sizeof(float);
 #define DSVG_LNB(TT, NV) hipLaunchKernelGGL((ln_bwd_kernel<TT, NV>), dim3(nb), dim3(256), lds, st, (const TT*)dy, \
                                             (const TT*)x, mean, rstd, gamma, (const TT*)res, (TT*)dx, workspace,  \
                                             (long long)rows, d, (TT*)dx_masked, drop_p, (const uint64_t*)seed, drop_site)
@@ -252,6 +150,11 @@
     else { dsvg_set_error("layernorm_bwd: bad dtype %d", dtype); return -1; }
 #undef DSVG_LNB
     DSVG_LAUNCH_CHECK("layernorm_bwd");
+    return dsvg_ln_bwd_reduce(workspace, nb, d, dgamma, dbeta, accumulate, st);
+}
+
+int dsvg_ln_bwd_reduce(const float* workspace, int nb, int32_t d, float* dgamma, float* dbeta, int32_t accumulate,
+                       hipStream_t st) {
     if (dbeta == dgamma + d)
         return dsvg_reduce_partials_strided(workspace, nb, 2 * (int64_t)d, 2 * (int64_t)d, dgamma, accumulate, st);
     int rc = 0;
diff --git a/deepsvg_amd/csrc/ln_bwd_body.h b/deepsvg_amd/csrc/ln_bwd_body.h
--- /dev/null
+++ b/deepsvg_amd/csrc/ln_bwd_body.h
@@ -0,0 +1,157 @@
+#pragma once
+#include "dsvg_common.h"
+
+constexpr int LN_MAXV_MAX = 4;
+constexpr int LN_MAX_BLOCKS = 1024;
+
+int dsvg_ln_bwd_grid(long long rows);
+int dsvg_ln_bwd_reduce(const float* workspace, int nb, int32_t d, float* dgamma, float* dbeta, int32_t accumulate,
+                       hipStream_t st);
+
+__host__ __device__ constexpr size_t ln_bwd_lds_floats(int d) { return (size_t)4 * 2 * (d / 4 + 1) * 4; }
+
+template <typename T, int LN_MAXV, int NVB>
+__device__ __forceinline__ void ln_bwd_body(const T* dy, const T* __restrict__ x, const float* __restrict__ mean,
+                                            const float* __restrict__ rstd, const float* __restrict__ gamma, const T* res,
+                                            T* dx, float* __restrict__ part, long long rows, int d, T* dxm, float drop_p,
+                                            const uint64_t* __restrict__ seed, uint32_t site, float* red_raw, unsigned bid,
+                                            unsigned nblocks, unsigned bstride) {
+#pragma clang fp contract(off)
+    const DropCtx dmc = drop_make(dxm ? drop_p : 0.f, seed, site);
+    const int nvec = d / 4 + 1;
+    auto red = [&](int w, int k, int vec, int e) -> float& { return red_raw[((w * 2 + k) * nvec + vec) * 4 + e]; };
+    const int lane = threadIdx.x & 63;
+    const int wave = threadIdx.x >> 6;
+    const int nv = d / 256 + ((d % 256) ? 1 : 0);
+    float ag[NVB][LN_MAXV][4], ab[NVB][LN_MAXV][4];
+#pragma unroll
+    for (int v = 0; v < NVB; ++v)
+#pragma unroll
+        for (int i = 0; i < LN_MAXV; ++i)
+#pragma unroll
+            for (int e = 0; e < 4; ++e) { ag[v][i][e] = 0.f; ab[v][i][e] = 0.f; }
+
+    float4 g4[LN_MAXV];
+#pragma unroll
+    for (int i = 0; i < LN_MAXV; ++i) g4[i] = *reinterpret_cast<const float4*>(gamma + min(i * 256 + lane * 4, d - 4));
+    long long rowv[NVB];
+#pragma unroll
+    for (int v = 0; v < NVB; ++v) rowv[v] = (bid + v * bstride < nblocks) ? (long long)(bid + v * bstride) * 4 + wave : rows;
+    for (long long row0 = (long long)bid * 4 + wave; row0 < rows; row0 += (long long)nblocks * 4) {
+        float mu[NVB], rs[NVB];
+        float xh[NVB][LN_MAXV][4], gd[NVB][LN_MAXV][4], rv[NVB][LN_MAXV][4];
+        float c1[NVB], c2[NVB];
+        bool live[NVB];
+#pragma unroll
+        for (int v = 0; v < NVB; ++v) {
+            live[v] = v == 0 || rowv[v] < rows;
+            const long long row = v == 0 ? row0 : (live[v] ? rowv[v] : row0);
+            mu[v] = mean[row];
+            rs[v] = rstd[row];
+            c1[v] = 0.f;
+            c2[v] = 0.f;
+#pragma unroll
+            for (int i = 0; i < LN_MAXV; ++i) {
+                const int c = i * 256 + lane * 4;
+                if (i < nv && c < d) {
+                    float xv[4], dv[4];
+                    Elem<T>::ld4(x + row * d + c, xv);
+                    Elem<T>::ld4(dy + row * d + c, dv);
+                    if (res) Elem<T>::ld4(res + row * d + c, rv[v][i]);
+                    const float4 g = g4[i];
+                    const float gg[4] = {g.x, g.y, g.z, g.w};
+#pragma unroll
+                    for (int e = 0; e < 4; ++e) {
+                        xh[v][i][e] = (xv[e] - mu[v]) * rs[v];
+                        gd[v][i][e] = gg[e] * dv[e];
+                        c1[v] += gd[v][i][e];
+                        c2[v] += gd[v][i][e] * xh[v][i][e];
+                        if (v == 0 || live[v]) {
+                            ag[v][i][e] = __builtin_fmaf(dv[e], xh[v][i][e], ag[v][i][e]);
+                            ab[v][i][e] += dv[e];
+                        }
+                    }
+                } else {
+#pragma unroll
+                    for (int e = 0; e < 4; ++e) { xh[v][i][e] = 0.f; gd[v][i][e] = 0.f; }
+                }
+            }
+        }
+#pragma unroll
+        for (int v = 0; v < NVB; ++v) {
+            c1[v] = wave_sum(c1[v]) / (float)d;
+            c2[v] = wave_sum(c2[v]) / (float)d;
+        }
+#pragma unroll
+        for (int v = 0; v < NVB; ++v) {
+            const long long row = v == 0 ? row0 : rowv[v];
+            if (v != 0 && !live[v]) continue;
+#pragma unroll
+            for (int i = 0; i < LN_MAXV; ++i) {
+                const int c = i * 256 + lane * 4;
+                if (i < nv && c < d) {
+                    float o[4];
+#pragma unroll
+                    for (int e = 0; e < 4; ++e) {
+                        const float t = __builtin_fmaf(-c2[v], xh[v][i][e], gd[v][i][e] - c1[v]);
+                        o[e] = res ? __builtin_fmaf(rs[v], t, rv[v][i][e]) : rs[v] * t;
+                    }
+                    Elem<T>::st4(dx + row * d + c, o);
+                    if (dxm) {
+                        const uint64_t id4 = (uint64_t)row * (uint64_t)d + (uint64_t)c;
+                        float mm[4] = {1.f, 1.f, 1.f, 1.f};
+                        if (dmc.on) {
+                            const uint32_t hg = drop_group(dmc, id4 >> 3);
+                            const uint32_t wb = ((uint32_t)id4 & 4u) ? 2u : 0u;
+                            const uint32_t w0 = drop_word(hg, wb), w1 = drop_word(hg, wb + 1u);
+                            mm[0] = (w0 & 0xffffu) < dmc.thresh ? 0.f : dmc.scale;
+                            mm[1] = (w0 >> 16) < dmc.thresh ? 0.f : dmc.scale;
+                            mm[2] = (w1 & 0xffffu) < dmc.thresh ? 0.f : dmc.scale;
+                            mm[3] = (w1 >> 16) < dmc.thresh ? 0.f : dmc.scale;
+                        }
+                        float om[4];
+#pragma unroll
+                        for (int e = 0; e < 4; ++e) {
+                            T t;
+                            Elem<T>::st(&t, o[e]);
+                            om[e] = Elem<T>::ld(&t) * mm[e];
+                        }
+                        Elem<T>::st4(dxm + row * d + c, om);
+                    }
+                }
+            }
+        }
+#pragma unroll
+        for (int v = 1; v < NVB; ++v) rowv[v] += (long long)nblocks * 4;
+    }
+    const int vstride = (int)ln_bwd_lds_floats(d);
+#pragma unroll
+    for (int v = 0; v < NVB; ++v) {
+#pragma unroll
+        for (int i = 0; i < LN_MAXV; ++i) {
+            if (i < nv) {
+#pragma unroll
+                for (int e = 0; e < 4; ++e) {
+                    if (i * 256 + lane * 4 < d) {
+                        (&red(wave, 0, i * 64 + lane, e))[v * vstride] = ag[v][i][e];
+                        (&red(wave, 1, i * 64 + lane, e))[v * vstride] = ab[v][i][e];
+                    }
+                }
+            }
+        }
+    }
+    __syncthreads();
+#pragma unroll
+    for (int v = 0; v < NVB; ++v) {
+        if (v != 0 && !(bid + v * bstride < nblocks)) continue;
+        float* pg = part + (size_t)(bid + v * bstride) * 2 * d;
+        for (int c = threadIdx.x; c < d; c += 256) {
+            const int vec = c >> 2, e = c & 3;
+            float sg = 0.f, sb = 0.f;
+#pragma unroll
+            for (int w = 0; w < 4; ++w) { sg += (&red(w, 0, vec, e))[v * vstride]; sb += (&red(w, 1, vec, e))[v * vstride]; }
+            pg[c] = sg;
+            pg[d + c] = sb;
+        }
+    }
+}
diff --git a/deepsvg_amd/functional.py b/deepsvg_amd/functional.py
--- a/deepsvg_amd/functional.py
+++ b/deepsvg_amd/functional.py
@@ -10,6 +10,10 @@
 FFN_MIN_ROWS = int(os.environ.get("DSVG_FFN_MIN_ROWS", "16384"))
 ATTN_MIN_ROWS = int(os.environ.get("DSVG_ATTN_MIN_ROWS", "16384"))
 FFN_GATE_DW2 = os.environ.get("DSVG_FFN_GATE_DW2", "1") != "0"
+
+WGRAD_LN = os.environ.get("DSVG_WGRAD_LN", "1") != "0"
+WGRAD_LN_MIN_ROWS = int(os.environ.get("DSVG_WGRAD_LN_MIN_ROWS", "16384"))
+WGRAD_LN_MIN_WGS = 257
 
 LN_BWD_MASKED = os.environ.get("DSVG_LN_BWD_MASKED", "1") != "0"
 DEFER_MORE = os.environ.get("DSVG_DEFER_MORE", "1") != "0"
@@ -120,6 +124,13 @@
             ops.gemm(dy, x, a_kc=False, b_kc=False, out=dw)
             ops.colsum(dy, out=db)
     return dw, db
+
+
+def _wgrad_ln_route(dy, x, weight, split, xin):
+    if not (WGRAD_LN and xin.is_cuda and xin.shape[0] >= WGRAD_LN_MIN_ROWS and xin.dtype == torch.bfloat16 and xin.shape[1] == 256):
+        return False
+    tiles = -(-weight.shape[0] // 128) * -(-weight.shape[1] // 128)
+    return tiles * split >= WGRAD_LN_MIN_WGS and ops.gemm_wgrad_ln_bwd_ok(dy, x, split, xin)
 
 
 def _group_blocks(w):
@@ -841,7 +852,10 @@
                 dqkv = ops.attention_bwd(qkv, key_mask, dao, n_seq, S, H, ctx.scale, p, s0, rt.seed, seq_off=seq_off,
                                          tiles=ctx.tiles, **_path_kw(rt, S))
         del dx1m
-        dwin, dbin = _wbgrad(rt, win, bin_, dqkv, xn1)
+        split_in = ops.split_k_for(*win.shape, dqkv.shape[0])
+        pair = _wgrad_ln_route(dqkv, xn1, win, split_in, x)
+        if not pair:
+            dwin, dbin = _wbgrad(rt, win, bin_, dqkv, xn1, split=split_in)
         dx_out = None
         if live is not None:
             dx_full = torch.empty((full_rows, x.shape[1]), dtype=x.dtype, device=x.device)
@@ -849,8 +863,14 @@
         mk = (p, ctx.mask_below, rt.seed) if (ctx.mask_below is not None and p > 0) else None
         with rt.deferring():
             dxn1 = ops.gemm(dqkv, rt.w(win), b_kc=False)
-            out = ops.layernorm_bwd(dxn1, x, mean1, rstd1, n1w.detach(), res=dx1, dx=dx_out,
-                                    dgamma=rt.grad_out(n1w), dbeta=rt.grad_out(n1b), masked=mk)
+            if pair:
+                dwin, dbin = rt.grad_out(win), rt.grad_out(bin_)
+                with _wgrad_tag():
+                    out = ops.gemm_wgrad_ln_bwd(dqkv, xn1, dwin, dbin, split_in, dxn1, x, mean1, rstd1, n1w.detach(), res=dx1,
+                                                dx=dx_out, dgamma=rt.grad_out(n1w), dbeta=rt.grad_out(n1b), masked=mk)[1:]
+            else:
+                out = ops.layernorm_bwd(dxn1, x, mean1, rstd1, n1w.detach(), res=dx1, dx=dx_out,
+                                        dgamma=rt.grad_out(n1w), dbeta=rt.grad_out(n1b), masked=mk)
             dx, dn1w, dn1b = out[:3]
         if live is not None:
             dx = dx_full
diff --git a/deepsvg_amd/lib.py b/deepsvg_amd/lib.py
--- a/deepsvg_amd/lib.py
+++ b/deepsvg_amd/lib.py
@@ -9,7 +9,7 @@
 DSVG_I64 = 2
 DSVG_RASTER_FILL, DSVG_RASTER_CULL = 1, 2
 DSVG_RASTER_WIDE = 4
-ABI_VERSION = 18
+ABI_VERSION = 19
 
 c_i32, c_i64, c_u32, c_f32 = C.c_int32, C.c_int64, C.c_uint32, C.c_float
 vp = C.c_void_p
@@ -64,6 +64,8 @@
     "dsvg_layernorm_bwd_workspace_bytes": (c_i64, [c_i64, c_i32]),
     "dsvg_layernorm_bwd_masked": (c_i32, [c_i32, vp, vp, vp, vp, vp, vp, vp, vp, vp, c_i32, c_i64, c_i32, vp, c_i64, vp, c_f32,
                                           c_u32, vp, vp]),
+    "dsvg_gemm_wgrad_ln_bwd": (c_i32, [C.POINTER(GemmDesc), c_i32, vp, vp, vp, vp, vp, vp, vp, vp, vp, c_i32, c_i64, c_i32, vp,
+                                       c_i64, vp, c_f32, c_u32, vp, vp]),
     "dsvg_attention_fwd": (c_i32, [c_i32, vp, vp, vp, c_i64, vp, vp, c_i64, c_i32, c_i32, c_f32, c_f32, c_u32, vp, vp]),
     "dsvg_attention_bwd": (c_i32, [c_i32, vp, vp, vp, c_i64, vp, vp, vp, c_i64, c_i32, c_i32, c_f32, c_f32, c_u32, vp, vp]),
     "dsvg_attention_tiles": (c_i32, [vp, c_i64, c_i32, vp, vp, vp]),
diff --git a/deepsvg_amd/ops.py b/deepsvg_amd/ops.py
--- a/deepsvg_amd/ops.py
+++ b/deepsvg_amd/ops.py
@@ -411,6 +411,50 @@
              "dsvg_layernorm_bwd")
     _prof_end(ev, 0.0, 0.0, dict(op="layernorm_bwd"))
     return dx, dgamma, dbeta
+
+
+def gemm_wgrad_ln_bwd_ok(a, b, split_k, dy):
+    return (split_k > 1 and a.is_cuda and a.dtype == b.dtype == dy.dtype == torch.bfloat16 and a.dim() == b.dim() == 2
+            and a.is_contiguous() and b.is_contiguous() and dy.is_contiguous() and dy.shape[1] == 256
+            and a.shape[0] == b.shape[0] and a.shape[0] % 64 == 0 and a.shape[1] % 8 == 0 and b.shape[1] % 8 == 0
+            and a.data_ptr() % 16 == 0 and b.data_ptr() % 16 == 0)
+
+
+def gemm_wgrad_ln_bwd(a, b, out, rowsum, split_k, dy, x, mean, rstd, gamma, *, res=None, dgamma=None, dbeta=None,
+                      accumulate=False, dx=None, masked=None):
+    _chk(a, b, out, rowsum, dy, x, mean, rstd, gamma, res, dgamma, dbeta)
+    d_, M, N, _odt, ws_bytes = _gemm_build(a, b, False, False, None, None, False, 0, None, 1.0, 0.0, 0, 0.0, 0, None, out, None,
+                                           False, split_k, 0, rowsum)
+    assert dy.is_contiguous() and x.is_contiguous() and dy.shape == x.shape
+    rows, d = x.shape
+    if dx is None:
+        dx = torch.empty_like(x)
+    if dgamma is None:
+        dgamma = torch.empty(d, dtype=torch.float32, device=x.device)
+    if dbeta is None:
+        dbeta = torch.empty(d, dtype=torch.float32, device=x.device)
+    if res is not None:
+        assert res.is_contiguous() and res.shape == x.shape and res.dtype == x.dtype
+    L = _l.load()
+    d_.A, d_.B, d_.C = a.data_ptr(), b.data_ptr(), out.data_ptr()
+    d_.rowsum = rowsum.data_ptr() if rowsum is not None else None
+    gws = _ws(ws_bytes, a.device)
+    d_.workspace, d_.workspace_bytes = gws.data_ptr(), gws.numel() * 4
+    ws = _ws(L.dsvg_layernorm_bwd_workspace_bytes(rows, d), x.device)
+    dxm, mp, msite, mseed = None, 0.0, 0, None
+    if masked is not None:
+        mp, msite, mseed = masked
+        dxm = torch.empty_like(dx)
+    ev = _prof_begin()
+    _l.check(L.dsvg_gemm_wgrad_ln_bwd(C.byref(d_), _dt(x), dy.data_ptr(), x.data_ptr(), mean.data_ptr(), rstd.data_ptr(),
+                                      gamma.data_ptr(), _p(res), dx.data_ptr(), dgamma.data_ptr(), dbeta.data_ptr(),
+                                      int(accumulate), rows, d, ws.data_ptr(), ws.numel() * 4, _p(dxm), float(mp), int(msite),
+                                      _p(mseed) if mp > 0 else None, _stream()), "dsvg_gemm_wgrad_ln_bwd")
+    _prof_end(ev, 2.0 * M * N * a.shape[0], float(2 * (a.numel() + b.numel()) + 4 * M * N),
+              dict(op="gemm_wgrad_ln_bwd", a=tuple(a.shape), b=tuple(b.shape), split_k=split_k, rows=rows))
+    if masked is not None:
+        return out, dx, dgamma, dbeta, dxm
+    return out, dx, dgamma, dbeta
 
 
 def attention_tiles(seq_off, n_seq, max_rows=32):
diff --git a/include/dsvg.h b/include/dsvg.h
--- a/include/dsvg.h
+++ b/include/dsvg.h
@@ -12,7 +12,7 @@
 #define DSVG_BF16 1
 #define DSVG_I64 2
 
-#define DSVG_ABI_VERSION 18
+#define DSVG_ABI_VERSION 19
 
 const char* dsvg_last_error(void);
 int dsvg_version(void);
@@ -63,6 +63,10 @@
                               const float* gamma, const void* res, void* dx, float* dgamma, float* dbeta,
                               int32_t accumulate, int64_t rows, int32_t d, float* workspace, int64_t workspace_bytes,
                               void* dx_masked, float drop_p, uint32_t drop_site, const void* seed, void* stream);
+int dsvg_gemm_wgrad_ln_bwd(const dsvg_gemm_desc* g, int32_t dtype, const void* dy, const void* x, const float* mean,
+                           const float* rstd, const float* gamma, const void* res, void* dx, float* dgamma, float* dbeta,
+                           int32_t accumulate, int64_t rows, int32_t d, float* workspace, int64_t workspace_bytes,
+                           void* dx_masked, float drop_p, uint32_t drop_site, const void* seed, void* stream);
 
 int dsvg_attention_fwd(int32_t dtype, const void* qkv, const uint64_t* key_mask, const int32_t* seq_off,
                        int64_t total_rows, const int32_t* tile_first, void* out, int64_t n_seq, int32_t S,
```

Result: no change. 94140 icons/s, median of 6 (+1.0%).
